# chzchzchz/raftsql

Measured on AMD Instinct MI355X. Metric: quorum decisions/sec (commit+vote) across G groups, higher is better.
Workload: dtype u64

## Files before the change

go/raftq/engine_more.go:

```go
package raftq

import "C"

import "unsafe"

func ABIVersion() int { return int(C.raftq_abi_version()) }

func Quorum(peers uint32) uint32 { return uint32(C.raftq_quorum(C.uint32_t(peers))) }

func (e *Engine) NGroups() uint64 { return uint64(C.raftq_groups(e.h)) }
func (e *Engine) NPeers() uint32  { return uint32(C.raftq_peers(e.h)) }

func (e *Engine) SelfMax() (int, error) {
	var slot C.int32_t
	if err := e.err(C.raftq_self_max(e.h, &slot)); err != nil {
		return -1, err
	}
	return int(slot), nil
}

func (e *Engine) Narrow() (bool, error) {
	var valid C.int32_t
	if err := e.err(C.raftq_narrow(e.h, &valid)); err != nil {
		return false, err
	}
	return valid != 0, nil
}

func (e *Engine) NarrowRebuild() error { return e.err(C.raftq_narrow_rebuild(e.h)) }

func (e *Engine) SetStream(stream unsafe.Pointer) error { return e.err(C.raftq_set_stream(e.h, stream)) }
func (e *Engine) Stream() unsafe.Pointer                { return C.raftq_get_stream(e.h) }

type TermDelta struct{ Group, CurTerm, FirstIdxCurTerm uint64 }

func (e *Engine) ApplyTermDeltas(d []TermDelta) error {
	if len(d) == 0 {
		return nil
	}
	return e.err(C.raftq_apply_term_deltas(e.h, (*C.raftq_term_delta_t)(unsafe.Pointer(&d[0])), C.uint64_t(len(d))))
}

func (e *Engine) CommitAdvance(gated bool, committedOut []uint64) (changed uint64, err error) {
	var p *C.uint64_t
	if committedOut != nil {
		p = (*C.uint64_t)(unsafe.Pointer(&committedOut[0]))
	}
	g := C.int(0)
	if gated {
		g = 1
	}
	var n C.uint64_t
	err = e.err(C.raftq_commit_advance(e.h, g, p, &n))
	return uint64(n), err
}

func (e *Engine) VoteTally(outcomeOut []uint8) (Counts, error) {
	var p *C.uint8_t
	if outcomeOut != nil {
		p = (*C.uint8_t)(unsafe.Pointer(&outcomeOut[0]))
	}
	var c C.raftq_counts_t
	if err := e.err(C.raftq_vote_tally(e.h, p, &c)); err != nil {
		return Counts{}, err
	}
	return Counts{uint64(c.n_changed), uint64(c.n_won), uint64(c.n_lost)}, nil
}

func (e *Engine) ReadVotes(out []uint8) error {
	return e.err(C.raftq_read_votes(e.h, (*C.uint8_t)(unsafe.Pointer(&out[0]))))
}

func (e *Engine) SetTimers(electionTick, heartbeatTick uint32, seed uint64) error {
	return e.err(C.raftq_set_timers(e.h, C.uint32_t(electionTick), C.uint32_t(heartbeatTick), C.uint64_t(seed)))
}

type TickCounts struct{ Hup, Beat uint64 }

func (e *Engine) Tick(wantCounts bool) (TickCounts, error) {
	var c C.raftq_tick_counts_t
	if !wantCounts {
		return TickCounts{}, e.err(C.raftq_tick(e.h, nil))
	}
	err := e.err(C.raftq_tick(e.h, &c))
	return TickCounts{uint64(c.n_hup), uint64(c.n_beat)}, err
}

func (e *Engine) CollectHups(out []uint64) (uint64, error) {
	var n C.uint64_t
	var p *C.uint64_t
	if len(out) > 0 {
		p = (*C.uint64_t)(unsafe.Pointer(&out[0]))
	}
	rc := C.raftq_collect_hups(e.h, p, C.uint64_t(len(out)), &n)
	return uint64(n), e.err(rc)
}

func (e *Engine) TickCollect(hups, beats []uint64) (nHup, nBeat uint64, err error) {
	var hp, bp *C.uint64_t
	if len(hups) > 0 {
		hp = (*C.uint64_t)(unsafe.Pointer(&hups[0]))
	}
	if len(beats) > 0 {
		bp = (*C.uint64_t)(unsafe.Pointer(&beats[0]))
	}
	var nh, nb C.uint64_t
	err = e.err(C.raftq_tick_collect(e.h, hp, C.uint64_t(len(hups)), &nh, bp, C.uint64_t(len(beats)), &nb))
	return uint64(nh), uint64(nb), err
}

const TickBeatBitmap = uint(C.RAFTQ_TICK_BEAT_BITMAP)

// ... 202 lines not shown
```

include/raftq.h:

```cpp
#ifndef RAFTQ_H
#define RAFTQ_H

#include <stddef.h>
#include <stdint.h>

#ifdef __cplusplus
extern "C" {
#endif

#define RAFTQ_ABI_VERSION 1
#define RAFTQ_MAX_PEERS 9

#define RAFTQ_OK 0
#define RAFTQ_EINVAL (-1)
#define RAFTQ_ENOMEM (-2)
#define RAFTQ_EHIP (-3)
#define RAFTQ_ESTATE (-4)
#define RAFTQ_ENODEV (-5)

#define RAFTQ_SWEEP_COMMIT 0x01u
#define RAFTQ_SWEEP_GATED 0x02u
#define RAFTQ_SWEEP_VOTES 0x04u
#define RAFTQ_SWEEP_NO_ADOPT 0x08u
#define RAFTQ_SWEEP_LDS 0x10u
// ... 16 lines not shown
  uint64_t match;
  uint32_t peer;
  uint32_t _pad;
} raftq_delta_t;

typedef struct raftq_vote_delta {
  uint64_t group;
  uint32_t peer;
  uint8_t vote;
  uint8_t _pad[3];
} raftq_vote_delta_t;

typedef struct raftq_term_delta {
  uint64_t group;
  uint64_t cur_term;
  uint64_t first_idx_cur_term;
} raftq_term_delta_t;

typedef struct raftq_advance {
  uint64_t group;
  uint64_t old_commit;
  uint64_t new_commit;
} raftq_advance_t;

typedef struct raftq_delta16 {
  uint64_t match;
  uint32_t group;
  uint32_t peer;
} raftq_delta16_t;
typedef struct raftq_advance16 {
  uint64_t new_commit;
  uint32_t group;
  uint32_t advanced_by;
} raftq_advance16_t;

int raftq_abi_version(void);
int raftq_device_count(int* n);
uint32_t raftq_quorum(uint32_t n_peers);

#define RAFTQ_MAX_GROUPS (1ull << 30)
int raftq_create(int device, uint64_t n_groups, uint32_t n_peers, raftq_t** out);
void raftq_destroy(raftq_t* h);
uint64_t raftq_groups(const raftq_t* h);
uint32_t raftq_peers(const raftq_t* h);
const char* raftq_last_error(const raftq_t* h);

int raftq_set_stream(raftq_t* h, void* stream);
void* raftq_get_stream(const raftq_t* h);

int raftq_load_match(raftq_t* h, const uint64_t* match ,
                     const uint64_t* committed );
int raftq_load_terms(raftq_t* h, const uint64_t* cur_term ,
                     const uint64_t* first_idx_cur_term );
int raftq_load_votes(raftq_t* h, const uint8_t* votes );

int raftq_apply_deltas(raftq_t* h, const raftq_delta_t* d, uint64_t n);
int raftq_apply_vote_deltas(raftq_t* h, const raftq_vote_delta_t* d, uint64_t n);
int raftq_apply_term_deltas(raftq_t* h, const raftq_term_delta_t* d, uint64_t n);

typedef struct raftq_voter_delta {
  uint64_t group;
  uint16_t voters;
  uint16_t reset;
  uint32_t _pad;
} raftq_voter_delta_t;
int raftq_load_voters(raftq_t* h, const uint16_t* voters);
int raftq_apply_voter_deltas(raftq_t* h, const raftq_voter_delta_t* d, uint64_t n);
int raftq_read_voters(raftq_t* h, uint16_t* voters_out);

int raftq_step_async(raftq_t* h, unsigned flags);
int raftq_wait(raftq_t* h, raftq_counts_t* counts);

int raftq_commit_advance(raftq_t* h, int gated, uint64_t* committed_out ,
                         uint64_t* n_changed );
int raftq_vote_tally(raftq_t* h, uint8_t* outcome_out ,
                     raftq_counts_t* counts );

int raftq_read_committed(raftq_t* h, uint64_t* committed_out );
int raftq_read_outcome(raftq_t* h, uint8_t* outcome_out );
int raftq_read_match(raftq_t* h, uint64_t* match_out );
int raftq_self_max(raftq_t* h, int32_t* slot_out);
int raftq_narrow(raftq_t* h, int32_t* valid_out);
int raftq_narrow_rebuild(raftq_t* h);
int raftq_read_votes(raftq_t* h, uint8_t* votes_out );
int raftq_collect_changed(raftq_t* h, raftq_advance_t* out, uint64_t cap, uint64_t* n);

#define RAFTQ_ROLE_FOLLOWER 0
#define RAFTQ_ROLE_CANDIDATE 1
#define RAFTQ_ROLE_LEADER 2
typedef struct raftq_tick_counts {
  uint64_t n_hup;
  uint64_t n_beat;
} raftq_tick_counts_t;
int raftq_set_timers(raftq_t* h, uint32_t election_tick, uint32_t heartbeat_tick, uint64_t seed);
int raftq_load_roles(raftq_t* h, const uint8_t* role , const uint32_t* elapsed );
int raftq_tick_set_voters(raftq_t* h, int on);
int raftq_tick(raftq_t* h, raftq_tick_counts_t* counts);
int raftq_read_tick(raftq_t* h, uint8_t* action , uint32_t* elapsed , uint8_t* role );
int raftq_collect_hups(raftq_t* h, uint64_t* groups, uint64_t cap, uint64_t* n);
int raftq_collect_beats(raftq_t* h, uint64_t* groups, uint64_t cap, uint64_t* n);
int raftq_tick_collect(raftq_t* h, uint64_t* hups, uint64_t hup_cap, uint64_t* n_hup, uint64_t* beats, uint64_t beat_cap,
                       uint64_t* n_beat);

#define RAFTQ_TICK_BEAT_BITMAP 1u
int raftq_tick_collect_lists(raftq_t* h, unsigned flags, uint64_t hup_cap, uint64_t beat_cap, uint64_t* n_hup, uint64_t* n_beat);
int raftq_last_tick_lists(raftq_t* h, const uint32_t** hups, uint64_t* n_hups, const uint32_t** beats, uint64_t* n_beats,
                          const uint64_t** beat_bitmap, uint64_t* bitmap_words);
int raftq_campaign(raftq_t* h, const uint64_t* groups, uint64_t n, uint32_t self_peer);

int raftq_cycle(raftq_t* h, const raftq_delta_t* deltas, uint64_t n_deltas,
                const raftq_vote_delta_t* vote_deltas, uint64_t n_vote_deltas, unsigned flags,
                raftq_advance_t* advances_out, uint64_t cap, uint64_t* n_advanced,
                raftq_counts_t* counts);

int raftq_stage(raftq_t* h, uint64_t n_deltas, uint64_t n_vote_deltas, raftq_delta_t** deltas,
                raftq_vote_delta_t** vote_deltas);
int raftq_last_advances(raftq_t* h, const raftq_advance_t** list, uint64_t* n_listed);

int raftq_cycle_packed(raftq_t* h, const raftq_delta16_t* deltas, uint64_t n_deltas,
                       const raftq_vote_delta_t* vote_deltas, uint64_t n_vote_deltas, unsigned flags,
                       raftq_advance16_t* advances_out, uint64_t cap, uint64_t* n_advanced,
                       raftq_counts_t* counts);
int raftq_stage_packed(raftq_t* h, uint64_t n_deltas, uint64_t n_vote_deltas, raftq_delta16_t** deltas,
                       raftq_vote_delta_t** vote_deltas);
int raftq_last_advances_packed(raftq_t* h, const raftq_advance16_t** list, uint64_t* n_listed);

#define RAFTQ_CYCLE_SEGMENTED 0x200u
int raftq_last_advance_segments(raftq_t* h, const raftq_advance16_t** recs, const uint32_t** counts, uint32_t* n_segments,
                                uint64_t* stride);

typedef struct raftq_set raftq_set_t;
#define RAFTQ_SET_GRID 0
#define RAFTQ_SET_PERSISTENT 1
int raftq_set_create(raftq_t* const* handles, uint32_t n, raftq_set_t** out);
void raftq_set_destroy(raftq_set_t* s);
uint32_t raftq_set_size(const raftq_set_t* s);
const char* raftq_set_last_error(const raftq_set_t* s);
void* raftq_set_get_stream(const raftq_set_t* s);
int raftq_set_mode(raftq_set_t* s, int mode, uint32_t persist_workgroups);
int raftq_set_sweep_async(raftq_set_t* s, unsigned flags);
int raftq_set_tick(raftq_set_t* s);
int raftq_set_wait(raftq_set_t* s, raftq_counts_t* per_member, raftq_counts_t* total);
int raftq_set_timer_begin(raftq_set_t* s);
int raftq_set_timer_end(raftq_set_t* s, float* elapsed_ms);
int raftq_sweep_many_async(raftq_t* const* handles, uint32_t n, unsigned flags);
int raftq_clone_state(raftq_t* dst, raftq_t* src);

int raftq_timer_begin(raftq_t* h);
int raftq_timer_end(raftq_t* h, float* elapsed_ms);

int raftq_host_alloc(void** p, uint64_t bytes);
void raftq_host_free(void* p);

#ifdef __cplusplus
}
#endif
#endif
```

raftsql_amd/_lib.py:

```python
from __future__ import annotations

import ctypes as C
import os

_HERE = os.path.dirname(os.path.abspath(__file__))
LIB_PATH = os.environ.get("RAFTQ_LIB") or os.path.join(_HERE, "libraftq.so")

RAFTQ_OK = 0
RAFTQ_EINVAL, RAFTQ_ENOMEM, RAFTQ_EHIP, RAFTQ_ESTATE, RAFTQ_ENODEV = -1, -2, -3, -4, -5

SWEEP_COMMIT = 0x01
SWEEP_GATED = 0x02
SWEEP_VOTES = 0x04
SWEEP_NO_ADOPT = 0x08
SWEEP_LDS = 0x10
SWEEP_CHANGED = 0x20
SWEEP_STREAM = 0x40
SWEEP_CACHED = 0x80
CYCLE_TRUSTED = 0x100
TICK_BEAT_BITMAP = 1
CYCLE_SEGMENTED = 0x200
SET_GRID, SET_PERSISTENT = 0, 1

MAX_PEERS = 9


class Counts(C.Structure):
    _fields_ = [("n_changed", C.c_uint64), ("n_won", C.c_uint64), ("n_lost", C.c_uint64)]


class TickCounts(C.Structure):
    _fields_ = [("n_hup", C.c_uint64), ("n_beat", C.c_uint64)]


class Delta(C.Structure):
    _fields_ = [("group", C.c_uint64), ("match", C.c_uint64), ("peer", C.c_uint32), ("_pad", C.c_uint32)]


class VoteDelta(C.Structure):
    _fields_ = [("group", C.c_uint64), ("peer", C.c_uint32), ("vote", C.c_uint8), ("_pad", C.c_uint8 * 3)]


class VoterDelta(C.Structure):
    _fields_ = [("group", C.c_uint64), ("voters", C.c_uint16), ("reset", C.c_uint16), ("_pad", C.c_uint32)]


class Advance(C.Structure):
    _fields_ = [("group", C.c_uint64), ("old_commit", C.c_uint64), ("new_commit", C.c_uint64)]


_H = C.c_void_p
_SIGS = [
    ("raftq_abi_version", C.c_int, []),
    ("raftq_device_count", C.c_int, [C.POINTER(C.c_int)]),
    ("raftq_quorum", C.c_uint32, [C.c_uint32]),
    ("raftq_create", C.c_int, [C.c_int, C.c_uint64, C.c_uint32, C.POINTER(_H)]),
    ("raftq_destroy", None, [_H]),
    ("raftq_groups", C.c_uint64, [_H]),
    ("raftq_peers", C.c_uint32, [_H]),
    ("raftq_last_error", C.c_char_p, [_H]),
    ("raftq_set_stream", C.c_int, [_H, C.c_void_p]),
    ("raftq_get_stream", C.c_void_p, [_H]),
    ("raftq_load_match", C.c_int, [_H, C.c_void_p, C.c_void_p]),
    ("raftq_load_terms", C.c_int, [_H, C.c_void_p, C.c_void_p]),
    ("raftq_load_votes", C.c_int, [_H, C.c_void_p]),
    ("raftq_apply_deltas", C.c_int, [_H, C.c_void_p, C.c_uint64]),
    ("raftq_apply_vote_deltas", C.c_int, [_H, C.c_void_p, C.c_uint64]),
    ("raftq_apply_term_deltas", C.c_int, [_H, C.c_void_p, C.c_uint64]),
    ("raftq_load_voters", C.c_int, [_H, C.c_void_p]),
    ("raftq_apply_voter_deltas", C.c_int, [_H, C.c_void_p, C.c_uint64]),
    ("raftq_read_voters", C.c_int, [_H, C.c_void_p]),
    ("raftq_step_async", C.c_int, [_H, C.c_uint]),
    ("raftq_wait", C.c_int, [_H, C.POINTER(Counts)]),
    ("raftq_commit_advance", C.c_int, [_H, C.c_int, C.c_void_p, C.POINTER(C.c_uint64)]),
    ("raftq_vote_tally", C.c_int, [_H, C.c_void_p, C.POINTER(Counts)]),
    ("raftq_read_committed", C.c_int, [_H, C.c_void_p]),
    ("raftq_read_outcome", C.c_int, [_H, C.c_void_p]),
    ("raftq_read_match", C.c_int, [_H, C.c_void_p]),
    ("raftq_self_max", C.c_int, [_H, C.POINTER(C.c_int32)]),
    ("raftq_narrow", C.c_int, [_H, C.POINTER(C.c_int32)]),
    ("raftq_narrow_rebuild", C.c_int, [_H]),
    ("raftq_read_votes", C.c_int, [_H, C.c_void_p]),
    ("raftq_collect_changed", C.c_int, [_H, C.c_void_p, C.c_uint64, C.POINTER(C.c_uint64)]),
    ("raftq_set_timers", C.c_int, [_H, C.c_uint32, C.c_uint32, C.c_uint64]),
    ("raftq_load_roles", C.c_int, [_H, C.c_void_p, C.c_void_p]),
    ("raftq_tick_set_voters", C.c_int, [_H, C.c_int]),
    ("raftq_tick", C.c_int, [_H, C.POINTER(TickCounts)]),
    ("raftq_read_tick", C.c_int, [_H, C.c_void_p, C.c_void_p, C.c_void_p]),
    ("raftq_collect_hups", C.c_int, [_H, C.c_void_p, C.c_uint64, C.POINTER(C.c_uint64)]),
    ("raftq_collect_beats", C.c_int, [_H, C.c_void_p, C.c_uint64, C.POINTER(C.c_uint64)]),
    ("raftq_tick_collect", C.c_int, [_H, C.c_void_p, C.c_uint64, C.POINTER(C.c_uint64), C.c_void_p, C.c_uint64, C.POINTER(C.c_uint64)]),
    ("raftq_tick_collect_lists", C.c_int, [_H, C.c_uint, C.c_uint64, C.c_uint64, C.POINTER(C.c_uint64), C.POINTER(C.c_uint64)]),
    ("raftq_last_tick_lists", C.c_int, [_H, C.POINTER(C.c_void_p), C.POINTER(C.c_uint64), C.POINTER(C.c_void_p), C.POINTER(C.c_uint64),
                                        C.POINTER(C.c_void_p), C.POINTER(C.c_uint64)]),
    ("raftq_campaign", C.c_int, [_H, C.c_void_p, C.c_uint64, C.c_uint32]),
    ("raftq_cycle", C.c_int, [_H, C.c_void_p, C.c_uint64, C.c_void_p, C.c_uint64, C.c_uint, C.c_void_p, C.c_uint64,
                              C.POINTER(C.c_uint64), C.POINTER(Counts)]),
    ("raftq_stage", C.c_int, [_H, C.c_uint64, C.c_uint64, C.POINTER(C.c_void_p), C.POINTER(C.c_void_p)]),
    ("raftq_last_advances", C.c_int, [_H, C.POINTER(C.c_void_p), C.POINTER(C.c_uint64)]),
    ("raftq_cycle_packed", C.c_int, [_H, C.c_void_p, C.c_uint64, C.c_void_p, C.c_uint64, C.c_uint, C.c_void_p, C.c_uint64,
                                     C.POINTER(C.c_uint64), C.POINTER(Counts)]),
    ("raftq_stage_packed", C.c_int, [_H, C.c_uint64, C.c_uint64, C.POINTER(C.c_void_p), C.POINTER(C.c_void_p)]),
    ("raftq_last_advances_packed", C.c_int, [_H, C.POINTER(C.c_void_p), C.POINTER(C.c_uint64)]),
    ("raftq_last_advance_segments", C.c_int, [_H, C.POINTER(C.c_void_p), C.POINTER(C.c_void_p), C.POINTER(C.c_uint32), C.POINTER(C.c_uint64)]),
    ("raftq_set_create", C.c_int, [C.POINTER(_H), C.c_uint32, C.POINTER(_H)]),
    ("raftq_set_destroy", None, [_H]),
    ("raftq_set_size", C.c_uint32, [_H]),
    ("raftq_set_last_error", C.c_char_p, [_H]),
    ("raftq_set_get_stream", C.c_void_p, [_H]),
    ("raftq_set_mode", C.c_int, [_H, C.c_int, C.c_uint32]),
    ("raftq_set_sweep_async", C.c_int, [_H, C.c_uint]),
    ("raftq_set_wait", C.c_int, [_H, C.c_void_p, C.POINTER(Counts)]),
    ("raftq_set_tick", C.c_int, [_H]),
    ("raftq_set_timer_begin", C.c_int, [_H]),
    ("raftq_set_timer_end", C.c_int, [_H, C.POINTER(C.c_float)]),
    ("raftq_sweep_many_async", C.c_int, [C.POINTER(_H), C.c_uint32, C.c_uint]),
    ("raftq_clone_state", C.c_int, [_H, _H]),
    ("raftq_timer_begin", C.c_int, [_H]),
    ("raftq_timer_end", C.c_int, [_H, C.POINTER(C.c_float)]),
    ("raftq_host_alloc", C.c_int, [C.POINTER(C.c_void_p), C.c_uint64]),
    ("raftq_host_free", None, [C.c_void_p]),
]
EXPORTS = [s[0] for s in _SIGS]


class StepCounts(C.Structure):
    _fields_ = [("n_msgs", C.c_uint64), ("n_groups_touched", C.c_uint64)]


_STEP_SIGS = [
    ("raftq_set_self", C.c_int, [_H, C.c_uint32]),
    ("raftq_load_node", C.c_int, [_H, C.c_void_p, C.c_void_p, C.c_void_p, C.c_void_p, C.c_void_p]),
    ("raftq_read_node", C.c_int, [_H, C.c_void_p, C.c_void_p, C.c_void_p, C.c_void_p, C.c_void_p, C.c_void_p]),
    ("raftq_step_batch", C.c_int, [_H, C.c_void_p, C.c_uint64, C.c_void_p, C.POINTER(StepCounts)]),
    ("raftq_apply_log_deltas", C.c_int, [_H, C.c_void_p, C.c_uint64, C.c_void_p]),
    ("raftq_apply_log_deltas_nowait", C.c_int, [_H, C.c_void_p, C.c_uint64]),
    ("raftq_step_submit", C.c_int, [_H, C.c_void_p, C.c_uint64]),
    ("raftq_step_collect", C.c_int, [_H, C.c_void_p, C.POINTER(StepCounts)]),
    ("raftq_step_stage", C.c_int, [_H, C.c_uint64, C.POINTER(C.c_void_p)]),
    ("raftq_step_stage_packed", C.c_int, [_H, C.c_uint64, C.POINTER(C.c_void_p)]),
    ("raftq_step_submit_packed", C.c_int, [_H, C.c_void_p, C.c_uint64]),
    ("raftq_step_results", C.c_int, [_H, C.POINTER(C.c_void_p), C.POINTER(C.c_uint64)]),
    ("raftq_step_set_compact", C.c_int, [_H, C.c_int]),
    ("raftq_step_set_msg_flags", C.c_int, [_H, C.c_int]),
    ("raftq_step_set_voters", C.c_int, [_H, C.c_int]),
    ("raftq_step_results_c", C.c_int, [_H, C.POINTER(C.c_void_p), C.POINTER(C.c_uint64)]),
    ("raftq_step_results_s", C.c_int, [_H, C.POINTER(C.c_void_p), C.POINTER(C.c_uint64)]),
]
STEP_EXPORTS = [s[0] for s in _STEP_SIGS]



class WireCounts(C.Structure):
    _fields_ = [("n_msgs", C.c_uint64), ("n_ents", C.c_uint64), ("n_malformed", C.c_uint64), ("bytes", C.c_uint64)]


class WalCounts(C.Structure):
    _fields_ = [("n_recs", C.c_uint64), ("n_valid", C.c_uint64), ("bytes", C.c_uint64), ("last_crc", C.c_uint32),
                ("_pad", C.c_uint32)]


_WIRE_SIGS = [
    ("raftq_wire_encode", C.c_int, [_H, C.c_void_p, C.c_uint64, C.c_void_p, C.c_uint64, C.c_void_p, C.c_uint64, C.c_void_p,
                                    C.c_uint64, C.c_void_p, C.POINTER(WireCounts)]),
# ... 67 lines not shown
```

raftsql_amd/csrc/raftq_capi.hip:

```cpp
#include "raftq.h"

#include <hip/hip_runtime.h>

#include <algorithm>
#include <atomic>
#include <mutex>
#include <chrono>
#include <cstdlib>
#include <cstdio>
#include <cstring>
#include <new>
#include <string>
#include <unordered_set>
#include <vector>

#include "raftq_internal.hpp"

#ifndef RAFTQ_GPL
#define RAFTQ_GPL 4
#endif
#ifndef RAFTQ_AUTO_STREAM_BYTES
#define RAFTQ_AUTO_STREAM_BYTES (128ull << 20)
#endif
#ifndef RAFTQ_LDS_GPL
// ... 134 lines not shown
template <int N>
hipError_t launch_voters_n(const VoterSweepArgs& a, uint64_t gpad, unsigned flags, int nt, hipStream_t s) {
  const bool commit = flags & (RAFTQ_SWEEP_COMMIT | RAFTQ_SWEEP_GATED);
  const bool gated = flags & RAFTQ_SWEEP_GATED;
  const bool votes = flags & RAFTQ_SWEEP_VOTES;
  if (commit && gated) return votes ? launch_voters_reg<N, true, true, true>(a, gpad, nt, s) : launch_voters_reg<N, true, true, false>(a, gpad, nt, s);
  if (commit) return votes ? launch_voters_reg<N, true, false, true>(a, gpad, nt, s) : launch_voters_reg<N, true, false, false>(a, gpad, nt, s);
  return launch_voters_reg<N, false, false, true>(a, gpad, nt, s);
}

hipError_t launch_voters(uint32_t N, const VoterSweepArgs& a, uint64_t gpad, unsigned flags, int nt, hipStream_t s) {
  switch (N) {
    case 1: return launch_voters_n<1>(a, gpad, flags, nt, s);
    case 2: return launch_voters_n<2>(a, gpad, flags, nt, s);
    case 3: return launch_voters_n<3>(a, gpad, flags, nt, s);
    case 4: return launch_voters_n<4>(a, gpad, flags, nt, s);
    case 5: return launch_voters_n<5>(a, gpad, flags, nt, s);
    case 6: return launch_voters_n<6>(a, gpad, flags, nt, s);
    case 7: return launch_voters_n<7>(a, gpad, flags, nt, s);
    case 8: return launch_voters_n<8>(a, gpad, flags, nt, s);
    case 9: return launch_voters_n<9>(a, gpad, flags, nt, s);
    default: return hipErrorInvalidValue;
  }
}

hipError_t launch_sweep(uint32_t N, const SweepLaunch& L, unsigned flags, int nt, hipStream_t s) {
  switch (N) {
    case 1: return launch_n<1>(L, flags, nt, s);
    case 2: return launch_n<2>(L, flags, nt, s);
    case 3: return launch_n<3>(L, flags, nt, s);
    case 4: return launch_n<4>(L, flags, nt, s);
    case 5: return launch_n<5>(L, flags, nt, s);
    case 6: return launch_n<6>(L, flags, nt, s);
    case 7: return launch_n<7>(L, flags, nt, s);
    case 8: return launch_n<8>(L, flags, nt, s);
    case 9: return launch_n<9>(L, flags, nt, s);
    default: return hipErrorInvalidValue;
  }
}

}
static inline void dense_changed(raftq_t* h) { h->node_mirror_fresh = false; }

int raftq_detail::ensure_staging(raftq_t* h, size_t bytes) {
  HIPCHK(h, h->stage.grow(bytes, std::max({bytes, h->stage.cap * 2, (size_t)1 << 20}), &h->stream));
  return RAFTQ_OK;
}

int raftq_detail::ensure_ingest(raftq_t* h, size_t bytes) {
  HIPCHK(h, h->ingest.grow(bytes, std::max({bytes, h->ingest.cap * 2, (size_t)1 << 20}), &h->stream, h->bar));
  return RAFTQ_OK;
}

namespace {
int ensure_adv(raftq_t* h, uint64_t entries) {
  const uint64_t have = h->adv.cap / sizeof(Advance);
  const uint64_t want = std::min<uint64_t>(std::max<uint64_t>({entries, have * 2, 4096}), h->gpad);
  HIPCHK(h, h->adv.grow(entries * sizeof(Advance), want * sizeof(Advance), &h->stream));
  return RAFTQ_OK;
}

}
int raftq_detail::self_max_check(raftq_t* h) {
  if (int rc = use_device(h)) return rc;
  if (h->step_collected != h->step_submitted) {
    HIPCHK(h, hipMemsetAsync(h->self_max, 0, sizeof(uint32_t), h->stream));
    return RAFTQ_OK;
  }
  HIPCHK(h, hipMemsetD32Async((hipDeviceptr_t)h->self_max, (int)(kSelfMaxValid | h->self_peer), 1, h->stream));
  const uint64_t blocks = std::min<uint64_t>((h->G + kBlock - 1) / kBlock, 4096);
  hipLaunchKernelGGL(self_max_check_kernel, dim3((unsigned)std::max<uint64_t>(blocks, 1)), dim3(kBlock), 0, h->stream,
                     (const uint64_t*)h->match, h->ld, h->G, h->N, h->self_peer, h->self_max);
  HIPCHK(h, hipGetLastError());
  return RAFTQ_OK;
}
int raftq_detail::narrow_build(raftq_t* h) {
  if (int rc = use_device(h)) return rc;
  if (h->narrow_off) return RAFTQ_OK;
  if (h->step_collected != h->step_submitted) {
    HIPCHK(h, hipMemsetAsync(h->narrow_word(), 0, sizeof(uint32_t), h->stream));
    return RAFTQ_OK;
  }
  if (!h->anchor) {
    const hipError_t e = raftq_buf::alloc_group({{(void**)&h->anchor, h->ld * sizeof(uint64_t)},
                                                 {(void**)&h->moff, (size_t)h->N * h->ld * sizeof(uint32_t)}},
                                                h->stream);
    if (e != hipSuccess) {
      (void)hipGetLastError();
      return RAFTQ_OK;
    }
    if (h->in_set) h->in_set->tab_stale = true;
  }
  HIPCHK(h, hipMemsetD32Async((hipDeviceptr_t)h->narrow_word(), (int)kNarrowValid, 1, h->stream));
  const uint64_t blocks = std::min<uint64_t>((h->G + kBlock - 1) / kBlock, 4096);
  hipLaunchKernelGGL(narrow_build_kernel, dim3((unsigned)std::max<uint64_t>(blocks, 1)), dim3(kBlock), 0, h->stream,
                     (const uint64_t*)h->match, h->ld, h->G, h->N, h->anchor, h->moff, h->narrow_word());
  HIPCHK(h, hipGetLastError());
  return RAFTQ_OK;
}
int raftq_detail::use_device(raftq_t* h) {
  if (!h) return fail(nullptr, RAFTQ_EINVAL, "null handle");
  HIPCHK(h, hipSetDevice(h->device));
  return RAFTQ_OK;
}
int raftq_detail::use_device_idle(raftq_t* h, const char* who) {
  if (int rc = use_device(h)) return rc;
  if (h->step_collected != h->step_submitted)
    return fail(h, RAFTQ_ESTATE, std::string(who) + ": Step batches are in flight; collect them first");
  return RAFTQ_OK;
}
using raftq_detail::ensure_staging;
using raftq_detail::ensure_ingest;
using raftq_detail::use_device;
using raftq_detail::use_device_idle;
using raftq_detail::ensure_tick_state;

template <typename W>
static void pack_votes(const uint8_t* votes, uint64_t G, uint32_t N, W* out) {
  for (uint64_t g = 0; g < G; ++g) out[g] = 0;
  for (uint32_t p = 0; p < N; ++p) {
    const uint8_t* row = votes + (size_t)p * G;
    for (uint64_t g = 0; g < G; ++g) {
      const uint8_t v = row[g];
      out[g] = (W)(out[g] | (W)((v == 1 ? 1u : v == 2 ? 2u : 0u) << (2 * p)));
    }
  }
}
template <typename W>
static void unpack_votes(const W* in, uint64_t G, uint32_t N, uint8_t* votes) {
  for (uint32_t p = 0; p < N; ++p) {
    uint8_t* row = votes + (size_t)p * G;
    for (uint64_t g = 0; g < G; ++g) {
      const uint32_t f = ((uint32_t)in[g] >> (2 * p)) & 3u;
      row[g] = f == 3u ? 0 : (uint8_t)f;
    }
  }
}

extern "C" {

int raftq_abi_version(void) { return RAFTQ_ABI_VERSION; }

uint32_t raftq_quorum(uint32_t n_peers) { return n_peers / 2 + 1; }

int raftq_device_count(int* n) {
  if (!n) return fail(nullptr, RAFTQ_EINVAL, "raftq_device_count: null out");
  int c = 0;
  hipError_t e = hipGetDeviceCount(&c);
  if (e != hipSuccess) {
    *n = 0;
    return fail(nullptr, RAFTQ_ENODEV, std::string("hipGetDeviceCount: ") + hipGetErrorString(e));
  }
  *n = c;
  return RAFTQ_OK;
}

const char* raftq_last_error(const raftq_t* h) { return h ? h->err.c_str() : g_err.c_str(); }

uint64_t raftq_groups(const raftq_t* h) { return h ? h->G : 0; }
uint32_t raftq_peers(const raftq_t* h) { return h ? h->N : 0; }

int raftq_create(int device, uint64_t n_groups, uint32_t n_peers, raftq_t** out) {
  if (!out) return fail(nullptr, RAFTQ_EINVAL, "raftq_create: null out");
  *out = nullptr;
  if (n_groups == 0 || n_groups > RAFTQ_MAX_GROUPS)
    return fail(nullptr, RAFTQ_EINVAL, "raftq_create: n_groups out of range (1 .. RAFTQ_MAX_GROUPS = 2^30 per handle)");
  if (n_peers < 1 || n_peers > RAFTQ_MAX_PEERS) return fail(nullptr, RAFTQ_EINVAL, "raftq_create: n_peers must be 1..9");
  int ndev = 0;
  if (hipGetDeviceCount(&ndev) != hipSuccess || ndev <= 0)
    return fail(nullptr, RAFTQ_ENODEV, "raftq_create: no HIP device (this library has no CPU path)");
  if (device < 0 || device >= ndev) return fail(nullptr, RAFTQ_ENODEV, "raftq_create: device index out of range");
  raftq_t* h = new (std::nothrow) raftq();
  if (!h) return fail(nullptr, RAFTQ_ENOMEM, "raftq_create: host allocation failed");
  h->device = device;
  h->G = n_groups;
  h->N = n_peers;
  h->last_gpl = kGPL;
  h->gpad = (n_groups + kTileMax - 1) / kTileMax * kTileMax;
  h->ld = h->gpad + kRowStagger;
  const uint64_t ld = h->ld;
  h->max_partials = h->gpad / (kBlock * 2) * kWaves;
  int rc = RAFTQ_OK;
  do {
    if ((rc = use_device(h))) break;
    hipError_t e = hipStreamCreateWithFlags(&h->stream, hipStreamNonBlocking);
    if (e != hipSuccess) { rc = fail(h, RAFTQ_EHIP, std::string("hipStreamCreate: ") + hipGetErrorString(e)); break; }
    h->own_stream = true;
    {
      int large_bar = 0;
      (void)hipDeviceGetAttribute(&large_bar, hipDeviceAttributeIsLargeBar, device);
      const char* st = std::getenv("RAFTQ_STAGE");
      h->bar.staging = large_bar == 1 && !(st && std::strcmp(st, "host") == 0);
    }
    e = raftq_buf::alloc_group({{(void**)&h->match, (size_t)n_peers * ld * 8},
                                {(void**)&h->committed[0], ld * 8},
                                {(void**)&h->committed[1], ld * 8},
                                {(void**)&h->first_idx, ld * 8},
                                {(void**)&h->votes, (size_t)vote_word_bytes((int)n_peers) * ld},
                                {(void**)&h->outcome, ld / 4 + 64},
                                {(void**)&h->changed_bits, h->gpad / 8},
                                {(void**)&h->partials, h->max_partials * sizeof(uint4)},
                                {(void**)&h->offsets, (h->max_partials + 1) * 8},
                                {(void**)&h->self_max, 64}},
                               h->stream);
    if (e != hipSuccess) {
      rc = fail(h, e == hipErrorOutOfMemory ? RAFTQ_ENOMEM : RAFTQ_EHIP, std::string("device arrays: ") + hipGetErrorString(e));
      break;
    }
    {
      const char* nr = std::getenv("RAFTQ_NARROW");
      h->narrow_off = nr && std::strcmp(nr, "0") == 0;
    }
    e = hipMemsetD32Async((hipDeviceptr_t)h->self_max, (int)(kSelfMaxValid | 0u), 1, h->stream);
    if (e != hipSuccess) { rc = fail(h, RAFTQ_EHIP, std::string("hipMemsetD32Async: ") + hipGetErrorString(e)); break; }
    e = raftq_buf::alloc_group({{(void**)&h->h_partials, h->max_partials * sizeof(uint4), raftq_buf::Kind::pinned},
                                {(void**)&h->h_total, 64, raftq_buf::Kind::mapped_coherent, (void**)&h->d_total}},
                               h->stream);
    if (e != hipSuccess) { rc = fail(h, RAFTQ_ENOMEM, std::string("page-locked memory: ") + hipGetErrorString(e)); break; }
    e = hipEventCreate(&h->ev0);
    if (e == hipSuccess) e = hipEventCreate(&h->ev1);
    if (e != hipSuccess) { rc = fail(h, RAFTQ_EHIP, std::string("hipEventCreate: ") + hipGetErrorString(e)); break; }
    e = hipStreamSynchronize(h->stream);
    if (e != hipSuccess) { rc = fail(h, RAFTQ_EHIP, std::string("hipStreamSynchronize: ") + hipGetErrorString(e)); break; }
  } while (0);
  if (rc != RAFTQ_OK) {
    std::string keep = h->err;
    raftq_destroy(h);
    g_err = keep;
    return rc;
  }
  *out = h;
  return RAFTQ_OK;
}

void raftq_destroy(raftq_t* h) {
  if (!h) return;
  if (h->in_set) {
    raftq_set_t* s = h->in_set;
    s->broken = true;
    s->members.erase(std::remove(s->members.begin(), s->members.end(), h), s->members.end());
    (void)hipSetDevice(h->device);
    (void)hipStreamSynchronize(s->stream);
    h->stream = nullptr;
    h->own_stream = false;
  }
  if (h->prof_n && std::getenv("RAFTQ_PROFILE"))
    std::fprintf(stderr,
                 "[raftq] cycle phases, avg us over %llu calls: stage/validate %.1f | enqueue scatter %.1f | enqueue sweep "
                 "%.1f | enqueue collect %.1f | sync %.1f | copy-out %.1f | turns that ended in the blocking wait instead of the "
                 "polled flag: %llu\n",
                 (unsigned long long)h->prof_n, h->prof[0] / h->prof_n, h->prof[1] / h->prof_n, h->prof[2] / h->prof_n,
                 h->prof[3] / h->prof_n, h->prof[4] / h->prof_n, h->prof[5] / h->prof_n, (unsigned long long)h->flag_fallbacks);
  (void)hipSetDevice(h->device);
  if (h->stream) (void)hipStreamSynchronize(h->stream);
  if (h->many_aux) (void)hipStreamSynchronize(h->many_aux);
  raftq_detail::free_node_state(h);
  raftq_detail::free_wire_state(h);
  raftq_buf::free_device(h->match, h->committed[0], h->committed[1], h->first_idx, h->votes, h->voters, h->outcome, h->changed_bits,
                         h->partials, h->offsets, h->self_max, h->anchor, h->moff, h->claim, h->delta_bad, h->role, h->elapsed, h->action, h->hup_bits,
                         h->beat_bits, h->tick_partials, h->tick_offsets2);
  raftq_buf::free_host(h->h_partials, h->h_total);
  if (h->ev0) (void)hipEventDestroy(h->ev0);
  if (h->ev1) (void)hipEventDestroy(h->ev1);
  if (h->many_aux) {
    (void)hipEventDestroy(h->many_fork);
    (void)hipEventDestroy(h->many_join);
  }
  const hipStream_t streams[4] = {h->many_aux, h->step_s_in, h->step_s_out, h->own_stream ? h->stream : nullptr};
  delete h;
  for (hipStream_t st : streams)
    if (st) (void)hipStreamDestroy(st);
}

int raftq_set_stream(raftq_t* h, void* stream) {
  if (int rc = use_device_idle(h, "raftq_set_stream")) return rc;
  if (h->in_set) return fail(h, RAFTQ_ESTATE, "raftq_set_stream: the handle is a member of a sweep set, which owns its stream");
  HIPCHK(h, hipStreamSynchronize(h->stream));
  if (h->own_stream) HIPCHK(h, hipStreamDestroy(h->stream));
  h->stream = (hipStream_t)stream;
  h->own_stream = false;
  return RAFTQ_OK;
}

void* raftq_get_stream(const raftq_t* h) { return h ? (void*)h->stream : nullptr; }

int raftq_load_match(raftq_t* h, const uint64_t* match, const uint64_t* committed) {
  if (int rc = use_device_idle(h, "raftq_load_match")) return rc;
  if (!match && !committed) return fail(h, RAFTQ_EINVAL, "raftq_load_match: nothing to load");
  if (match) {
    for (uint32_t p = 0; p < h->N; ++p)
      HIPCHK(h, hipMemcpyAsync(h->match + (size_t)p * h->ld, match + (size_t)p * h->G, h->G * 8, hipMemcpyHostToDevice, h->stream));
    if (int rc = raftq_detail::self_max_check(h)) return rc;
    if (int rc = raftq_detail::narrow_build(h)) return rc;
  }
  dense_changed(h);
  if (committed)
    HIPCHK(h, hipMemcpyAsync(h->committed[h->cur], committed, h->G * 8, hipMemcpyHostToDevice, h->stream));
  HIPCHK(h, hipStreamSynchronize(h->stream));
  return RAFTQ_OK;
}

int raftq_load_terms(raftq_t* h, const uint64_t* cur_term, const uint64_t* first_idx_cur_term) {
  if (int rc = use_device_idle(h, "raftq_load_terms")) return rc;
  if (!cur_term || !first_idx_cur_term) return fail(h, RAFTQ_EINVAL, "raftq_load_terms: null argument");
  std::vector<uint64_t> f;
  try {
    f.assign(first_idx_cur_term, first_idx_cur_term + h->G);
  } catch (...) {
    return fail(h, RAFTQ_ENOMEM, "raftq_load_terms: host allocation failed");
  }
  for (uint64_t g = 0; g < h->G; ++g)
    if (cur_term[g] == 0) f[g] = 0;
  HIPCHK(h, hipMemcpyAsync(h->first_idx, f.data(), h->G * 8, hipMemcpyHostToDevice, h->stream));
  dense_changed(h);
  HIPCHK(h, hipStreamSynchronize(h->stream));
  h->have_terms = true;
  return RAFTQ_OK;
}

int raftq_load_votes(raftq_t* h, const uint8_t* votes) {
  if (int rc = use_device_idle(h, "raftq_load_votes")) return rc;
  if (!votes) return fail(h, RAFTQ_EINVAL, "raftq_load_votes: null argument");
  const size_t wb = (size_t)vote_word_bytes((int)h->N);
  std::vector<uint8_t> packed;
  try {
    packed.resize(h->G * wb);
  } catch (...) {
    return fail(h, RAFTQ_ENOMEM, "raftq_load_votes: host allocation failed");
  }
  if (wb == 2) pack_votes(votes, h->G, h->N, reinterpret_cast<uint16_t*>(packed.data()));
  else pack_votes(votes, h->G, h->N, reinterpret_cast<uint32_t*>(packed.data()));
  HIPCHK(h, hipMemcpyAsync(h->votes, packed.data(), packed.size(), hipMemcpyHostToDevice, h->stream));
  HIPCHK(h, hipStreamSynchronize(h->stream));
  return RAFTQ_OK;
}

static int ensure_delta_dev(raftq_t* h, size_t bytes) {
  if (!h->delta_bad) HIPCHK(h, raftq_buf::alloc_zeroed((void**)&h->delta_bad, 64, h->stream));
  HIPCHK(h, h->delta_dev.grow(bytes, std::max(bytes * 2, (size_t)1 << 20), &h->stream));
  return RAFTQ_OK;
}

static int check_deltas(raftq_t* h, bool trusted = false) {
  int rc = RAFTQ_OK;
  const char* what = trusted ? "; that record was dropped, every other record of the turn was applied (RAFTQ_CYCLE_TRUSTED)"
                             : "; nothing applied";
  if (h->delta_check[0] && h->h_total[1] == h->delta_check[0])
    rc = fail(h, RAFTQ_EINVAL, std::string("a match delta is out of range (group >= G or peer >= N)") + what);
  if (h->delta_check[1] && h->h_total[2] == h->delta_check[1])
    rc = fail(h, RAFTQ_EINVAL, std::string("a vote delta is invalid (group/peer out of range or vote not 1/2)") + what);
  h->delta_check[0] = h->delta_check[1] = 0;
  return rc;
}

}

template <typename Rec, typename AbiRec>
static int enqueue_ingest(raftq_t* h, const AbiRec* d, uint64_t n, const raftq_vote_delta_t* vd, uint64_t nv, size_t off_votes,
                          bool trusted = false) {
  static_assert(sizeof(Rec) == sizeof(AbiRec), "ABI struct mismatch");
  static_assert(sizeof(VoteDeltaRec) == sizeof(raftq_vote_delta_t), "ABI struct mismatch");
  if (nv > 0xfffffffeull) return fail(h, RAFTQ_EINVAL, "vote delta batch too large");
  auto inside = [&](const void* q) {
    return (const uint8_t*)q >= (const uint8_t*)h->ingest.h && (const uint8_t*)q < (const uint8_t*)h->ingest.h + h->ingest.cap;
  };
  if (n) {
    AbiRec* dst = (AbiRec*)h->ingest.h;
    if ((const void*)d != (const void*)dst) {
      if (inside(d)) return fail(h, RAFTQ_EINVAL, "match deltas staged with other counts / another record layout than this call's");
      std::memcpy(dst, d, (size_t)n * sizeof(AbiRec));
    }
  }
  if (nv) {
    raftq_vote_delta_t* dst = (raftq_vote_delta_t*)((uint8_t*)h->ingest.h + off_votes);
    if ((const void*)vd != (const void*)dst) {
      if (inside(vd)) return fail(h, RAFTQ_EINVAL, "vote deltas staged with other counts / another record layout than this call's");
      std::memcpy(dst, vd, (size_t)nv * sizeof(raftq_vote_delta_t));
    }
    if (!h->claim) {
      HIPCHK(h, raftq_buf::alloc_filled((void**)&h->claim, (size_t)h->N * h->ld * sizeof(uint32_t), 0xff, h->stream));
    }
  }
  h->ingest.publish();
  if (int rc = ensure_delta_dev(h, h->ingest.cap)) return rc;
  const unsigned long long em = n ? ++h->delta_epoch : kNoEpoch, ev = nv ? ++h->delta_epoch : kNoEpoch;
  h->delta_check[0] = n ? em : 0;
  h->delta_check[1] = nv ? ev : 0;
  Rec* dev_m = (Rec*)h->delta_dev.d;
  VoteDeltaRec* dev_v = (VoteDeltaRec*)((uint8_t*)h->delta_dev.d + off_votes);
  const unsigned long long* bad = h->delta_bad;
  const dim3 gm((unsigned)((n + kBlock - 1) / kBlock)), gv((unsigned)((nv + kBlock - 1) / kBlock));
  if (n) dense_changed(h);
  if (n && trusted)
    hipLaunchKernelGGL((deltas_in_apply_kernel<Rec>), gm, dim3(kBlock), 0, h->stream, (const Rec*)h->ingest.d, n, h->match, h->ld,
                       h->G, h->N, h->delta_bad, h->d_total + 1, em, h->self_max, h->narrow_mirror());
  else if (n)
    hipLaunchKernelGGL((deltas_in_kernel<Rec>), gm, dim3(kBlock), 0, h->stream, (const Rec*)h->ingest.d, dev_m, n, h->G, h->N,
                       h->delta_bad, h->d_total + 1, em);
  if (nv)
    hipLaunchKernelGGL(vote_deltas_in_kernel, gv, dim3(kBlock), 0, h->stream,
                       (const VoteDeltaRec*)((uint8_t*)h->ingest.d + off_votes), dev_v, nv, h->G, h->N, h->delta_bad + 1,
                       h->d_total + 2, ev);
  if (n && !trusted)
    hipLaunchKernelGGL((apply_deltas_kernel<Rec>), gm, dim3(kBlock), 0, h->stream, h->match, h->ld, (const Rec*)dev_m, n, bad, em,
                       ev, h->self_max, h->narrow_mirror());
  if (nv) {
    const unsigned long long em_gate = trusted ? kNoEpoch : em;
    hipLaunchKernelGGL(vote_claim_kernel, gv, dim3(kBlock), 0, h->stream, h->claim, h->ld, (const VoteDeltaRec*)dev_v, nv, bad,
                       em_gate, ev, h->G, h->N, trusted ? 1 : 0);
    hipLaunchKernelGGL(vote_apply_kernel, gv, dim3(kBlock), 0, h->stream, h->votes, h->N > 8 ? 1 : 0, h->claim, h->ld,
                       (const VoteDeltaRec*)dev_v, nv, bad, em_gate, ev, h->G, h->N, trusted ? 1 : 0);
  }
  HIPCHK(h, hipGetLastError());
  return RAFTQ_OK;
}

extern "C" {

int raftq_apply_deltas(raftq_t* h, const raftq_delta_t* d, uint64_t n) {
  if (int rc = use_device_idle(h, "raftq_apply_deltas")) return rc;
  if (n == 0) return RAFTQ_OK;
  if (!d) return fail(h, RAFTQ_EINVAL, "raftq_apply_deltas: null argument");
  if (int rc = ensure_ingest(h, (size_t)n * sizeof(raftq_delta_t))) return rc;
  if (int rc = enqueue_ingest<DeltaRec>(h, d, n, nullptr, 0, 0)) return rc;
  HIPCHK(h, hipStreamSynchronize(h->stream));
  return check_deltas(h);
}

int raftq_apply_term_deltas(raftq_t* h, const raftq_term_delta_t* d, uint64_t n) {
  static_assert(sizeof(TermDeltaRec) == sizeof(raftq_term_delta_t), "ABI struct mismatch");
  if (int rc = use_device_idle(h, "raftq_apply_term_deltas")) return rc;
  if (n == 0) return RAFTQ_OK;
  if (!d) return fail(h, RAFTQ_EINVAL, "raftq_apply_term_deltas: null argument");
  for (uint64_t i = 0; i < n; ++i)
    if (d[i].group >= h->G) return fail(h, RAFTQ_EINVAL, "a term delta is out of range; nothing applied");
  if (int rc = ensure_staging(h, (size_t)n * sizeof(raftq_term_delta_t))) return rc;
  raftq_term_delta_t* dst = (raftq_term_delta_t*)h->stage.h;
  uint64_t m = 0;
  {
    std::unordered_set<uint64_t> seen;
    seen.reserve((size_t)n * 2);
    std::vector<uint64_t> keep;
    keep.reserve(n);
    for (uint64_t i = n; i-- > 0;)
      if (seen.insert(d[i].group).second) keep.push_back(i);
    for (auto it = keep.rbegin(); it != keep.rend(); ++it) dst[m++] = d[*it];
  }
  const dim3 grid((unsigned)((m + kBlock - 1) / kBlock));
  dense_changed(h);
  hipLaunchKernelGGL(apply_term_deltas_kernel, grid, dim3(kBlock), 0, h->stream, h->first_idx,
                     (const TermDeltaRec*)h->stage.d, m);
  HIPCHK(h, hipGetLastError());
  HIPCHK(h, hipStreamSynchronize(h->stream));
  h->have_terms = true;
  return RAFTQ_OK;
}

int raftq_apply_vote_deltas(raftq_t* h, const raftq_vote_delta_t* d, uint64_t n) {
  if (int rc = use_device_idle(h, "raftq_apply_vote_deltas")) return rc;
  if (n == 0) return RAFTQ_OK;
  if (!d) return fail(h, RAFTQ_EINVAL, "raftq_apply_vote_deltas: null argument");
  if (int rc = ensure_ingest(h, (size_t)n * sizeof(raftq_vote_delta_t))) return rc;
  if (int rc = enqueue_ingest<DeltaRec>(h, (const raftq_delta_t*)nullptr, 0, d, n, 0)) return rc;
  HIPCHK(h, hipStreamSynchronize(h->stream));
  return check_deltas(h);
}

}

static int ensure_voters(raftq_t* h) {
  if (h->voters) return RAFTQ_OK;
  HIPCHK(h, raftq_buf::alloc_zeroed((void**)&h->voters, h->ld * sizeof(uint16_t), h->stream));
  return RAFTQ_OK;
}
static int drop_voters(raftq_t* h) {
  if (!h->voters) return RAFTQ_OK;
  HIPCHK(h, hipStreamSynchronize(h->stream));
  raftq_buf::free_device(h->voters);
  return RAFTQ_OK;
}
static int voters_not_in_set(raftq_t* h, const char* who) {
  if (!h->in_set) return RAFTQ_OK;
  return fail(h, RAFTQ_ESTATE, std::string(who) + ": the handle is a member of a sweep set, whose dispatches count every slot "
                                                  "(voter masks on set members are out of scope)");
}
int raftq_detail::refuse_voters(raftq_t* h, const char* who, bool step_family, bool tick_rounds, bool bcast) {
  if (!h || !h->voters) return RAFTQ_OK;
  if (tick_rounds && h->tick_voters) return RAFTQ_OK;
  if (bcast) {
    if (h->bcast_voters) return RAFTQ_OK;
    return fail(h, RAFTQ_ESTATE, std::string(who) + ": the handle has voter masks loaded and did not opt in with raftq_bcast_set_voters; its broadcast "
                                                    "would go to N - 1 slots, not to a group's membership (whatever raftq_step_set_voters and "
                                                    "raftq_tick_set_voters say)");
  }
  if (h->step_voters) {
    if (step_family) return RAFTQ_OK;
    return fail(h, RAFTQ_ESTATE, std::string(who) + ": the handle has voter masks loaded; the broadcasts built on the device go to N - 1 slots, "
                                                    "not to a group's membership (out of scope, whatever raftq_step_set_voters says)");
  }
  return fail(h, RAFTQ_ESTATE, std::string(who) + ": the handle has voter masks loaded; Step's maybeCommit / poll on the device "
                                                  "count every slot (out of scope: raftq_load_voters(h, NULL) first)");
}

extern "C" {

int raftq_load_voters(raftq_t* h, const uint16_t* voters) {
  if (int rc = use_device_idle(h, "raftq_load_voters")) return rc;
  if (int rc = voters_not_in_set(h, "raftq_load_voters")) return rc;
  if (!voters) return drop_voters(h);
  const uint32_t beyond = 0xffffu & ~((1u << h->N) - 1u);
  for (uint64_t g = 0; g < h->G; ++g)
    if (voters[g] & beyond) return fail(h, RAFTQ_EINVAL, "raftq_load_voters: a mask names a peer slot >= N; nothing loaded");
  if (int rc = ensure_voters(h)) return rc;
  HIPCHK(h, hipMemcpyAsync(h->voters, voters, h->G * sizeof(uint16_t), hipMemcpyHostToDevice, h->stream));
  HIPCHK(h, hipStreamSynchronize(h->stream));
  return RAFTQ_OK;
}

int raftq_read_voters(raftq_t* h, uint16_t* voters_out) {
  if (int rc = use_device_idle(h, "raftq_read_voters")) return rc;
  if (!voters_out) return fail(h, RAFTQ_EINVAL, "raftq_read_voters: null argument");
  if (!h->voters) {
    std::fill(voters_out, voters_out + h->G, (uint16_t)((1u << h->N) - 1u));
    return RAFTQ_OK;
  }
  HIPCHK(h, hipMemcpyAsync(voters_out, h->voters, h->G * sizeof(uint16_t), hipMemcpyDeviceToHost, h->stream));
  HIPCHK(h, hipStreamSynchronize(h->stream));
  return RAFTQ_OK;
}

int raftq_apply_voter_deltas(raftq_t* h, const raftq_voter_delta_t* d, uint64_t n) {
  static_assert(sizeof(VoterDeltaRec) == sizeof(raftq_voter_delta_t), "ABI struct mismatch");
  if (int rc = use_device_idle(h, "raftq_apply_voter_deltas")) return rc;
  if (int rc = voters_not_in_set(h, "raftq_apply_voter_deltas")) return rc;
// ... 134 lines not shown
    return RAFTQ_OK;
  }
  raftq_t* h0 = handles[0];
  if (int rc = use_device(h0)) return rc;
  if (!h0->many_aux) {
    HIPCHK(h0, hipStreamCreateWithFlags(&h0->many_aux, hipStreamNonBlocking));
    HIPCHK(h0, hipEventCreateWithFlags(&h0->many_fork, hipEventDisableTiming));
    HIPCHK(h0, hipEventCreateWithFlags(&h0->many_join, hipEventDisableTiming));
  }
  HIPCHK(h0, hipEventRecord(h0->many_fork, h0->stream));
  HIPCHK(h0, hipStreamWaitEvent(h0->many_aux, h0->many_fork, 0));
  int rc = RAFTQ_OK;
  for (uint32_t i = 0; i < n && rc == RAFTQ_OK; ++i)
    rc = sweep_on(handles[i], flags, (i & 1) ? h0->many_aux : h0->stream, "raftq_sweep_many_async");
  HIPCHK(h0, hipEventRecord(h0->many_join, h0->many_aux));
  HIPCHK(h0, hipStreamWaitEvent(h0->stream, h0->many_join, 0));
  return rc;
}

int raftq_wait(raftq_t* h, raftq_counts_t* counts) {
  if (int rc = use_device_idle(h, "raftq_wait")) return rc;
  if (counts) {
    if (h->n_partials == 0) return fail(h, RAFTQ_ESTATE, "raftq_wait: no sweep to report on");
    HIPCHK(h, hipMemcpyAsync(h->h_partials, h->partials, h->n_partials * sizeof(uint4), hipMemcpyDeviceToHost, h->stream));
  }
  HIPCHK(h, hipStreamSynchronize(h->stream));
  if (counts) {
    uint64_t c = 0, w = 0, l = 0;
    for (uint64_t i = 0; i < h->n_partials; ++i) {
      c += h->h_partials[i].x;
      w += h->h_partials[i].y;
      l += h->h_partials[i].z;
    }
    const bool commit = h->last_flags & (RAFTQ_SWEEP_COMMIT | RAFTQ_SWEEP_GATED);
    const bool votes = h->last_flags & RAFTQ_SWEEP_VOTES;
    counts->n_changed = commit ? c : 0;
    counts->n_won = votes ? w : 0;
    counts->n_lost = votes ? l : 0;
  }
  return RAFTQ_OK;
}

int raftq_read_committed(raftq_t* h, uint64_t* out) {
  if (int rc = use_device_idle(h, "raftq_read_committed")) return rc;
  if (!out) return fail(h, RAFTQ_EINVAL, "raftq_read_committed: null argument");
  const uint64_t* src = (h->last_flags & RAFTQ_SWEEP_NO_ADOPT) && h->last_new ? h->last_new : h->committed[h->cur];
  HIPCHK(h, hipMemcpyAsync(out, src, h->G * 8, hipMemcpyDeviceToHost, h->stream));
  HIPCHK(h, hipStreamSynchronize(h->stream));
  return RAFTQ_OK;
}

int raftq_read_outcome(raftq_t* h, uint8_t* out) {
  if (int rc = use_device_idle(h, "raftq_read_outcome")) return rc;
  if (!out) return fail(h, RAFTQ_EINVAL, "raftq_read_outcome: null argument");
  std::vector<uint8_t> packed;
  try {
    packed.resize((h->G + 3) / 4);
  } catch (...) {
    return fail(h, RAFTQ_ENOMEM, "raftq_read_outcome: host allocation failed");
  }
  HIPCHK(h, hipMemcpyAsync(packed.data(), h->outcome, packed.size(), hipMemcpyDeviceToHost, h->stream));
  HIPCHK(h, hipStreamSynchronize(h->stream));
  for (uint64_t g = 0; g < h->G; ++g) out[g] = (uint8_t)((packed[g >> 2] >> (2 * (g & 3))) & 3u);
  return RAFTQ_OK;
}

int raftq_self_max(raftq_t* h, int32_t* slot) {
  if (int rc = use_device_idle(h, "raftq_self_max")) return rc;
  if (!slot) return fail(h, RAFTQ_EINVAL, "raftq_self_max: null argument");
  uint32_t w = 0;
  HIPCHK(h, hipMemcpyAsync(&w, h->self_max, sizeof w, hipMemcpyDeviceToHost, h->stream));
  HIPCHK(h, hipStreamSynchronize(h->stream));
  *slot = (w & kSelfMaxValid) ? (int32_t)(w & 0xffu) : -1;
  return RAFTQ_OK;
}

int raftq_narrow(raftq_t* h, int32_t* valid) {
  if (int rc = use_device_idle(h, "raftq_narrow")) return rc;
  if (!valid) return fail(h, RAFTQ_EINVAL, "raftq_narrow: null argument");
  uint32_t w = 0;
  HIPCHK(h, hipMemcpyAsync(&w, h->narrow_word(), sizeof w, hipMemcpyDeviceToHost, h->stream));
  HIPCHK(h, hipStreamSynchronize(h->stream));
  *valid = w == kNarrowValid ? 1 : 0;
  return RAFTQ_OK;
}

int raftq_narrow_rebuild(raftq_t* h) {
  if (int rc = use_device_idle(h, "raftq_narrow_rebuild")) return rc;
  if (int rc = raftq_detail::narrow_build(h)) return rc;
  HIPCHK(h, hipStreamSynchronize(h->stream));
  return RAFTQ_OK;
}

int raftq_read_match(raftq_t* h, uint64_t* out) {
  if (int rc = use_device_idle(h, "raftq_read_match")) return rc;
  if (!out) return fail(h, RAFTQ_EINVAL, "raftq_read_match: null argument");
  for (uint32_t p = 0; p < h->N; ++p)
    HIPCHK(h, hipMemcpyAsync(out + (size_t)p * h->G, h->match + (size_t)p * h->ld, h->G * 8, hipMemcpyDeviceToHost, h->stream));
  HIPCHK(h, hipStreamSynchronize(h->stream));
  return RAFTQ_OK;
}

int raftq_read_votes(raftq_t* h, uint8_t* out) {
  if (int rc = use_device_idle(h, "raftq_read_votes")) return rc;
  if (!out) return fail(h, RAFTQ_EINVAL, "raftq_read_votes: null argument");
  const size_t wb = (size_t)vote_word_bytes((int)h->N);
  std::vector<uint8_t> packed;
  try {
    packed.resize(h->G * wb);
  } catch (...) {
    return fail(h, RAFTQ_ENOMEM, "raftq_read_votes: host allocation failed");
  }
  HIPCHK(h, hipMemcpyAsync(packed.data(), h->votes, packed.size(), hipMemcpyDeviceToHost, h->stream));
  HIPCHK(h, hipStreamSynchronize(h->stream));
  if (wb == 2) unpack_votes(reinterpret_cast<const uint16_t*>(packed.data()), h->G, h->N, out);
  else unpack_votes(reinterpret_cast<const uint32_t*>(packed.data()), h->G, h->N, out);
  return RAFTQ_OK;
}

int raftq_commit_advance(raftq_t* h, int gated, uint64_t* committed_out, uint64_t* n_changed) {
  if (int rc = raftq_step_async(h, gated ? (RAFTQ_SWEEP_COMMIT | RAFTQ_SWEEP_GATED) : RAFTQ_SWEEP_COMMIT)) return rc;
  raftq_counts_t c;
  if (int rc = raftq_wait(h, &c)) return rc;
  if (n_changed) *n_changed = c.n_changed;
  if (committed_out) return raftq_read_committed(h, committed_out);
  return RAFTQ_OK;
}

int raftq_vote_tally(raftq_t* h, uint8_t* outcome_out, raftq_counts_t* counts) {
  if (int rc = raftq_step_async(h, RAFTQ_SWEEP_VOTES)) return rc;
  raftq_counts_t c;
  if (int rc = raftq_wait(h, &c)) return rc;
  if (counts) *counts = c;
  if (outcome_out) return raftq_read_outcome(h, outcome_out);
  return RAFTQ_OK;
}

}

int raftq_detail::ensure_tick_state(raftq_t* h) {
  if (h->role) return RAFTQ_OK;
  HIPCHK(h, raftq_buf::alloc_group({{(void**)&h->role, h->ld},
                                    {(void**)&h->elapsed, h->ld * 4},
                                    {(void**)&h->action, h->ld},
                                    {(void**)&h->hup_bits, h->gpad / 8},
                                    {(void**)&h->beat_bits, h->gpad / 8},
                                    {(void**)&h->tick_partials, h->gpad / 256 * sizeof(uint4)}},
                                   h->stream));
  return RAFTQ_OK;
}

static int ensure_tick_offsets2(raftq_t* h, uint64_t nw);
static hipError_t wait_turn(raftq_t* h, uint64_t flag_epoch, int kind = 0);

extern "C" {

int raftq_set_timers(raftq_t* h, uint32_t election_tick, uint32_t heartbeat_tick, uint64_t seed) {
  if (!h) return fail(nullptr, RAFTQ_EINVAL, "null handle");
  if (election_tick == 0 || heartbeat_tick == 0)
    return fail(h, RAFTQ_EINVAL, "raftq_set_timers: ticks must be >= 1");
  h->election_tick = election_tick;
  h->heartbeat_tick = heartbeat_tick;
  h->tick_seed = seed;
  return RAFTQ_OK;
}

// ... 899 lines not shown
  for (raftq_t* h : s->members) {
    h->tl_valid = false;
    ++h->tick_no;
    h->ticked = true;
  }
  return RAFTQ_OK;
}

int raftq_set_wait(raftq_set_t* s, raftq_counts_t* per_member, raftq_counts_t* total) {
  if (int rc = set_ready(s, "raftq_set_wait")) return rc;
  const bool want = per_member || total;
  const size_t n = s->members.size();
  if (want) {
    if (!s->swept) return sfail(s, RAFTQ_ESTATE, "raftq_set_wait: no set sweep to report on");
    set_fill_table(s, -1, s->tab_host);
    SETCHK(s, hipMemcpyAsync(s->tab[2], s->tab_host.data(), n * sizeof(SweepArgs), hipMemcpyHostToDevice, s->stream));
    s->np_host.resize(n);
    for (size_t i = 0; i < n; ++i) s->np_host[i] = s->members[i]->n_partials;
    SETCHK(s, hipMemcpyAsync(s->np_d, s->np_host.data(), n * 8, hipMemcpyHostToDevice, s->stream));
    hipLaunchKernelGGL(set_counts_kernel, dim3((unsigned)n), dim3(kBlock), 0, s->stream, (const SweepArgs*)s->tab[2],
                       (const uint64_t*)s->np_d, s->counts_d);
    SETCHK(s, hipGetLastError());
    SETCHK(s, hipMemcpyAsync(s->counts_h, s->counts_d, n * 32, hipMemcpyDeviceToHost, s->stream));
  }
  SETCHK(s, hipStreamSynchronize(s->stream));
  if (want) {
    raftq_counts_t t{0, 0, 0};
    for (size_t i = 0; i < n; ++i) {
      const unsigned f = s->members[i]->last_flags;
      const bool commit = f & (RAFTQ_SWEEP_COMMIT | RAFTQ_SWEEP_GATED);
      const bool votes = f & RAFTQ_SWEEP_VOTES;
      raftq_counts_t c{commit ? s->counts_h[4 * i] : 0, votes ? s->counts_h[4 * i + 1] : 0, votes ? s->counts_h[4 * i + 2] : 0};
      if (per_member) per_member[i] = c;
      t.n_changed += c.n_changed;
      t.n_won += c.n_won;
      t.n_lost += c.n_lost;
    }
    if (total) *total = t;
  }
  return RAFTQ_OK;
}

int raftq_set_timer_begin(raftq_set_t* s) {
  if (int rc = set_ready(s, "raftq_set_timer_begin")) return rc;
  SETCHK(s, hipEventRecord(s->ev0, s->stream));
  return RAFTQ_OK;
}

int raftq_set_timer_end(raftq_set_t* s, float* elapsed_ms) {
  if (int rc = set_ready(s, "raftq_set_timer_end")) return rc;
  if (!elapsed_ms) return sfail(s, RAFTQ_EINVAL, "raftq_set_timer_end: null argument");
  SETCHK(s, hipEventRecord(s->ev1, s->stream));
  SETCHK(s, hipEventSynchronize(s->ev1));
  SETCHK(s, hipEventElapsedTime(elapsed_ms, s->ev0, s->ev1));
  return RAFTQ_OK;
}

int raftq_clone_state(raftq_t* dst, raftq_t* src) {
  if (int rc = use_device_idle(dst, "raftq_clone_state")) return rc;
  if (!src) return fail(dst, RAFTQ_EINVAL, "raftq_clone_state: null source");
  if (src == dst) return RAFTQ_OK;
  if (src->device != dst->device || src->N != dst->N || src->G != dst->G)
    return fail(dst, RAFTQ_EINVAL, "raftq_clone_state: source and destination must have the same device, groups and peers");
  if (src->step_collected != src->step_submitted)
    return fail(dst, RAFTQ_ESTATE, "raftq_clone_state: the source has Step batches in flight");
  if (src->voters && dst->in_set)
    return fail(dst, RAFTQ_ESTATE, "raftq_clone_state: the source has voter masks loaded and the destination is a member of a sweep "
                                   "set, whose dispatches count every slot (out of scope)");
  if (src->voters) {
    if (int rc = ensure_voters(dst)) return rc;
  } else if (int rc = drop_voters(dst)) {
    return rc;
  }
  HIPCHK(dst, hipStreamSynchronize(src->stream));
  const uint64_t ld = dst->ld;
  HIPCHK(dst, hipMemcpyAsync(dst->match, src->match, (size_t)dst->N * ld * 8, hipMemcpyDeviceToDevice, dst->stream));
  HIPCHK(dst, hipMemcpyAsync(dst->committed[dst->cur], src->committed[src->cur], ld * 8, hipMemcpyDeviceToDevice, dst->stream));
  HIPCHK(dst, hipMemcpyAsync(dst->first_idx, src->first_idx, ld * 8, hipMemcpyDeviceToDevice, dst->stream));
  HIPCHK(dst, hipMemcpyAsync(dst->votes, src->votes, (size_t)vote_word_bytes((int)dst->N) * ld, hipMemcpyDeviceToDevice,
                             dst->stream));
  HIPCHK(dst, hipMemcpyAsync(dst->self_max, src->self_max, sizeof(uint32_t), hipMemcpyDeviceToDevice, dst->stream));
  if (src->anchor && !dst->narrow_off && !dst->anchor) {
    if (raftq_buf::alloc_group({{(void**)&dst->anchor, ld * sizeof(uint64_t), raftq_buf::Kind::device, nullptr, false},
                                {(void**)&dst->moff, (size_t)dst->N * ld * sizeof(uint32_t), raftq_buf::Kind::device, nullptr, false}},
                               dst->stream) != hipSuccess)
      (void)hipGetLastError();
    else if (dst->in_set) dst->in_set->tab_stale = true;
  }
  if (src->anchor && dst->anchor && !dst->narrow_off) {
    HIPCHK(dst, hipMemcpyAsync(dst->anchor, src->anchor, ld * sizeof(uint64_t), hipMemcpyDeviceToDevice, dst->stream));
    HIPCHK(dst, hipMemcpyAsync(dst->moff, src->moff, (size_t)dst->N * ld * sizeof(uint32_t), hipMemcpyDeviceToDevice, dst->stream));
    HIPCHK(dst, hipMemcpyAsync(dst->narrow_word(), src->narrow_word(), sizeof(uint32_t), hipMemcpyDeviceToDevice, dst->stream));
  } else {
    HIPCHK(dst, hipMemsetAsync(dst->narrow_word(), 0, sizeof(uint32_t), dst->stream));
  }
  if (src->voters) HIPCHK(dst, hipMemcpyAsync(dst->voters, src->voters, ld * sizeof(uint16_t), hipMemcpyDeviceToDevice, dst->stream));
  HIPCHK(dst, hipStreamSynchronize(dst->stream));
  dst->have_terms = src->have_terms;
  dense_changed(dst);
  return RAFTQ_OK;
}

}
```

raftsql_amd/csrc/raftq_internal.hpp:

```cpp
#pragma once
#include <hip/hip_runtime.h>

#include <string>
#include <vector>

#include "raftq.h"
#include "raftq_wire.h"
#include "raftq_kernels.hpp"
#include "raftq_buffers.hpp"

struct raftq {
  int device = 0;
  uint64_t G = 0, gpad = 0, ld = 0;
  uint32_t N = 0;
  hipStream_t stream = nullptr;
  bool own_stream = false;
  struct raftq_set* in_set = nullptr;
  uint64_t* match = nullptr;
  uint64_t* committed[2] = {nullptr, nullptr};
  int cur = 0;
  uint64_t* first_idx = nullptr;
  uint8_t* votes = nullptr;
  uint16_t* voters = nullptr;
  uint8_t* outcome = nullptr;
  uint64_t* changed_bits = nullptr;
  uint4* partials = nullptr;
  uint4* h_partials = nullptr;
  uint64_t n_partials = 0;
  uint64_t max_partials = 0;
  uint64_t* offsets = nullptr;
  uint64_t* h_total = nullptr;
  raftq_buf::Buffer<> stage{raftq_buf::Kind::mapped};
  raftq_buf::HostWritable ingest;
  raftq_buf::BarRule bar;
  std::vector<uint64_t> ld_mark, ld_start;
  struct LdNowait {
    raftq_buf::Buffer<> buf{raftq_buf::Kind::mapped};
    hipEvent_t ev = nullptr;
  };
  LdNowait ld_nowait[2];
  uint32_t ld_nowait_next = 0;
  std::vector<uint32_t> ld_round, ld_pos;
  uint32_t ld_epoch = 0;
  raftq_buf::Buffer<raftqk::Advance> adv{raftq_buf::Kind::mapped_coherent};
  uint64_t adv_listed = 0;
  bool adv_packed = false;
  bool adv_segmented = false;
  raftq_buf::Buffer<uint32_t> seg_h{raftq_buf::Kind::mapped_coherent};
  raftq_buf::Buffer<unsigned int> seg_d{raftq_buf::Kind::device};
  uint32_t seg_tiles = 0, seg_stride = 0, seg_one = 0;
  uint64_t flag_mask = ~0ull;
  uint32_t* self_max = nullptr;
  uint64_t* anchor = nullptr;
  uint32_t* moff = nullptr;
  bool narrow_off = false;
  uint32_t* narrow_word() const { return self_max + 1; }
  raftqk::NarrowMirror narrow_mirror() const { return raftqk::NarrowMirror{self_max + 1, anchor, moff}; }
  uint64_t compact_epoch = 0;
  uint64_t compact_epoch_armed = 0;
  uint32_t flag_misses[2] = {0, 0}, flag_rested[2] = {0, 0};
  uint64_t flag_fallbacks = 0;
  uint32_t* claim = nullptr;
  raftq_buf::Buffer<> delta_dev{raftq_buf::Kind::device};
  unsigned long long* delta_bad = nullptr;
  unsigned long long delta_epoch = 0;
  unsigned long long delta_check[2] = {0, 0};
  uint8_t* role = nullptr;
  uint32_t* elapsed = nullptr;
  uint8_t* action = nullptr;
  uint64_t* hup_bits = nullptr;
  uint64_t* beat_bits = nullptr;
  uint4* tick_partials = nullptr;
  raftq_buf::Buffer<uint32_t> tl{raftq_buf::Kind::mapped_coherent};
  uint64_t tl_hup_cap = 0, tl_beat_cap = 0, tl_beat_at = 0, tl_map_off = 0;
  uint64_t tl_n_hup = 0, tl_n_beat = 0;
  unsigned tl_flags = 0;
  bool tl_valid = false;
  uint64_t* tick_offsets2 = nullptr;
  uint32_t election_tick = 10, heartbeat_tick = 1;
  uint64_t tick_seed = 0x1000, tick_no = 0;
  bool ticked = false;
  uint64_t* d_total = nullptr;
  bool have_terms = false;
  unsigned last_flags = 0;
  int last_gpl = 0;
  const uint64_t* last_old = nullptr;
  const uint64_t* last_new = nullptr;
  uint32_t self_peer = 0;
  bool self_set = false;
  bool node_mirror_fresh = false;
  uint64_t node_mirror_refreshes = 0;
  void* node_rec = nullptr;
  unsigned int* step_stall = nullptr;
  uint8_t step_compact = 0;
  bool step_msg_flags = false;
  bool step_voters = false;
  bool tick_voters = false;
  bool bcast_voters = false;
  int step_walk_mode = 1;
  uint32_t step_stalls_in_a_row = 0, step_sorted_left = 0;
  uint64_t step_replays = 0;
  static constexpr int kStepSlots = 3;
  struct StepSlot {
    raftq_buf::Buffer<> in_h{raftq_buf::Kind::pinned};
    raftq_buf::HostWritable in_bar;
    raftq_buf::Buffer<> dev{raftq_buf::Kind::device};
    raftq_buf::Buffer<> out{raftq_buf::Kind::mapped};
    uint64_t n = 0;
    hipEvent_t ev_in = nullptr, ev_out = nullptr;
    bool busy = false;
    bool lists = false;
    bool replayed = false;
    bool copy_pending = false;
    const void* w_off_in_place = nullptr;
    const void* w_stream_in_place = nullptr;
    size_t w_stage_stream_off = 0;
    const void* msgs_in_place = nullptr;
    const void* outs_d = nullptr;
    uint64_t out_quads = 0;
    int end_bit = 0;
    uint32_t rec = 64;
    bool tail_zeroed = false;
    uint64_t tail_n = 0;
    uint32_t tail_rec = 0;
    const void* tail_dev = nullptr;
    uint64_t w_nbytes = 0;
    bool wire = false;
    uint8_t recs = 0;
    void* w_msgs_d = nullptr;
    void* w_ents_d = nullptr;
    const uint64_t* w_ent_total_d = nullptr;
    uint64_t w_ents_cap = 0;
    raftq_buf::Buffer<> w_pin{raftq_buf::Kind::pinned};
    bool w_msgs_fetched = false, w_ents_fetched = false;
    uint64_t w_n_ents = 0;
  } step_slot[kStepSlots];
  int step_last_slot = -1;
  uint64_t step_submitted = 0, step_collected = 0;
  hipStream_t step_s_in = nullptr, step_s_out = nullptr;
  bool step_defer_copy = true;
  const void* step_last_out = nullptr;
  uint64_t step_last_n = 0;
  uint32_t step_last_rec = 64;
  hipEvent_t ev0 = nullptr, ev1 = nullptr;
  hipStream_t many_aux = nullptr;
  hipEvent_t many_fork = nullptr, many_join = nullptr;
  raftq_buf::Buffer<> wire_dev{raftq_buf::Kind::device};
  raftq_buf::Buffer<> wire_out{raftq_buf::Kind::device};
  uint64_t* wire_pin = nullptr;
  uint64_t* wire_pin_d = nullptr;
  unsigned long long* wire_flags = nullptr;
  raftq_buf::Buffer<unsigned long long> wire_lb{raftq_buf::Kind::device};
  uint64_t wire_lb_tiles = 0;
  uint32_t wire_ticket_base = 0, wire_epoch = 0;
  uint32_t wire_chunk_base = 0, wire_chunk_pending = 0;
  bool wire_chunk_unknown = false;
  unsigned int prop_stamp = 0;
  raftq_buf::Buffer<> resp_dev{raftq_buf::Kind::device};
  bool resp_on = false;
  uint32_t resp_stamp = 0;
  const uint64_t* resp_at_tail_d = nullptr;
  bool wal_pending = false, wal_pending_done = false;
  bool wal_pending_waited = false;
  uint64_t wal_pending_n = 0, wal_pending_cap = 0;
  uint32_t wal_pending_prev = 0;
  int wal_pending_rc = 0;
  raftq_wal_counts_t wal_pending_counts{};
  std::string wal_pending_err;
  std::string err;
  double prof[6] = {0, 0, 0, 0, 0, 0};
  uint64_t prof_n = 0;
};


struct raftq_set {
  int device = 0;
  uint32_t N = 0;
  uint64_t gpad = 0;
  std::vector<raftq_t*> members;
  hipStream_t stream = nullptr;
  raftqk::SweepArgs* tab[3] = {nullptr, nullptr, nullptr};
  std::vector<raftqk::SweepArgs> tab_host;
  uint64_t* counts_d = nullptr;
  uint64_t* np_d = nullptr;
  std::vector<uint64_t> np_host;
  uint64_t* counts_h = nullptr;
  bool swept = false;
  bool broken = false;
  bool tab_stale = false;
  unsigned last_flags = 0;
  int mode = 0;
  uint32_t persist_wgs = 0;
  hipEvent_t ev0 = nullptr, ev1 = nullptr;
  raftqk::TickArgs* tick_tab = nullptr;
  std::vector<raftqk::TickArgs> tick_host;
  uint64_t tick_since = 0;
  std::string err;
};


struct raftq_wire_counts;
namespace raftqk {
struct NodeArrays;
}
namespace raftq_detail {
int node_arrays_of(raftq_t* h, raftqk::NodeArrays* out);
int fail(raftq_t* h, int code, const std::string& msg);
int use_device(raftq_t* h);
int use_device_idle(raftq_t* h, const char* who);
int refuse_voters(raftq_t* h, const char* who, bool step_family = false, bool tick_rounds = false, bool bcast = false);
inline bool masked_tick(const raftq_t* h) { return h->voters != nullptr && h->tick_voters; }
inline bool masked_bcast(const raftq_t* h) { return h->voters != nullptr && h->bcast_voters; }
int self_max_check(raftq_t* h);
int narrow_build(raftq_t* h);
int ensure_staging(raftq_t* h, size_t bytes);
int ensure_ingest(raftq_t* h, size_t bytes);
int ensure_tick_state(raftq_t* h);
void free_node_state(raftq_t* h);
void free_wire_state(raftq_t* h);
struct PackedDst {
  int form;
  uint32_t head_types;
  void* wide;
  uint64_t wide_cap;
};
int wire_frames_enqueue(raftq_t* h, const void* stream, uint64_t nbytes, const uint64_t* frame_off, uint64_t n, void* msgs, void* ents,
                        uint64_t ents_cap, void* msgs_d, int tail_appends, void* zero2 ,
                        const PackedDst* packed = nullptr);
uint64_t wire_frames_n_wide(raftq_t* h);
int wire_frames_finish(raftq_t* h, const uint64_t* frame_off, uint64_t n, bool have_ents, uint64_t ents_cap, ::raftq_wire_counts* counts);
struct RespPlan {
  uint64_t n = 0, n_max = 0, cap = 0;
  void* v_out = nullptr;
  uint64_t* v_resp_off = nullptr;
  uint64_t* peer_off = nullptr;
};
int respond_prepare(raftq_t* h, const void* stream, uint64_t nbytes, const uint64_t* frame_off, const void* msgs, const void* ents,
                    const uint64_t* at_tail, void* out, uint64_t cap, uint64_t* resp_off, uint64_t* peer_off, uint64_t n, RespPlan* p);
int respond_enqueue(raftq_t* h, const RespPlan& p);
int respond_finish(raftq_t* h, const RespPlan& p, ::raftq_wire_counts* resp_counts);
struct TickLists {
  unsigned flags;
  uint64_t cap_h, cap_b, beat_at, map_off;
  const uint64_t* off_beat;
  const uint64_t* off_h = nullptr;
};
int tick_lists_prepare(raftq_t* h, const char* who, unsigned flags, uint64_t hup_cap, uint64_t beat_cap, TickLists* tl);
int tick_lists_enqueue(raftq_t* h, TickLists* tl);
int tick_lists_finish(raftq_t* h, const char* who, const TickLists& tl, uint64_t* n_hup, uint64_t* n_beat);
int node_records_of(raftq_t* h, const char* who, raftqk::NodeArrays* out, bool tick_rounds = false, bool bcast = false);
int respond_pass_ok(raftq_t* h);
hipError_t wait_call(raftq_t* h);
}

#define HIPCHK(h, expr)                                                                        \
  do {                                                                                         \
    hipError_t _e = (expr);                                                                    \
    if (_e != hipSuccess) {                                                                    \
      return raftq_detail::fail((h), _e == hipErrorOutOfMemory ? RAFTQ_ENOMEM : RAFTQ_EHIP,    \
                                std::string(#expr) + ": " + hipGetErrorString(_e));            \
    }                                                                                          \
  } while (0)
```

raftsql_amd/csrc/raftq_kernels.hpp:

```cpp
#pragma once
#include <hip/hip_runtime.h>
#include <stdint.h>

#include <utility>

namespace raftqk {

typedef unsigned long long u64x2 __attribute__((ext_vector_type(2)));

constexpr int kBlock = 256;
constexpr int kWaves = kBlock / 64;
constexpr int kMaxPeers = 9;
constexpr int kTileMax = 2048;

struct SweepArgs {
  const uint64_t* match;
  const uint64_t* committed;
  uint64_t* committed_out;
  const uint64_t* first_idx;
  const uint8_t* votes;
  uint8_t* outcome;
  uint64_t* changed_bits;
  uint4* partials;
  uint64_t ld;
  const uint32_t* self_max = nullptr;
  const uint32_t* narrow = nullptr;
  const uint64_t* anchor = nullptr;
  const uint32_t* moff = nullptr;
};

constexpr uint32_t kSelfMaxValid = 0x80000000u;

constexpr uint32_t kNarrowValid = 1u;

template <typename T>
__device__ __forceinline__ void ce_desc(T& a, T& b) {
  const bool gt = a > b;
  const T hi = gt ? a : b;
  const T lo = gt ? b : a;
  a = hi;
  b = lo;
}

template <int N, typename T = uint64_t>
__device__ __forceinline__ T select_quorum_network(T (&v)[N]) {
#define CE(i, j) ce_desc(v[i], v[j])
  if constexpr (N == 2) { CE(0, 1); }
  if constexpr (N == 3) { CE(0, 2); CE(0, 1); CE(1, 2); }
  if constexpr (N == 4) { CE(0, 2); CE(1, 3); CE(0, 1); CE(2, 3); CE(1, 2); }
  if constexpr (N == 5) {
    CE(0, 3); CE(1, 4); CE(0, 2); CE(1, 3); CE(0, 1); CE(2, 4); CE(1, 2); CE(3, 4); CE(2, 3);
  }
  if constexpr (N == 6) {
    CE(0, 5); CE(1, 3); CE(2, 4); CE(1, 2); CE(3, 4); CE(0, 3);
    CE(2, 5); CE(0, 1); CE(2, 3); CE(4, 5); CE(1, 2); CE(3, 4);
  }
  if constexpr (N == 7) {
    CE(0, 6); CE(2, 3); CE(4, 5); CE(0, 2); CE(1, 4); CE(3, 6); CE(0, 1); CE(2, 5);
    CE(3, 4); CE(1, 2); CE(4, 6); CE(2, 3); CE(4, 5); CE(1, 2); CE(3, 4); CE(5, 6);
  }
  if constexpr (N == 8) {
    CE(0, 2); CE(1, 3); CE(4, 6); CE(5, 7); CE(0, 4); CE(1, 5); CE(2, 6); CE(3, 7); CE(0, 1); CE(2, 3);
    CE(4, 5); CE(6, 7); CE(2, 4); CE(3, 5); CE(1, 4); CE(3, 6); CE(1, 2); CE(3, 4); CE(5, 6);
  }
  if constexpr (N == 9) {
    CE(0, 3); CE(1, 7); CE(2, 5); CE(4, 8); CE(0, 7); CE(2, 4); CE(3, 8); CE(5, 6); CE(0, 2);
    CE(1, 3); CE(4, 5); CE(7, 8); CE(1, 4); CE(3, 6); CE(5, 7); CE(0, 1); CE(2, 4); CE(3, 5);
    CE(6, 8); CE(2, 3); CE(4, 5); CE(6, 7); CE(1, 2); CE(3, 4); CE(5, 6);
  }
#undef CE
  return v[N / 2];
}

template <int N>
__device__ __forceinline__ uint64_t select_other_network(uint64_t (&v)[N]) {
#define CE(i, j) ce_desc(v[i], v[j])
  if constexpr (N == 3) { CE(0, 1); }
  if constexpr (N == 4) { CE(0, 2); CE(0, 1); CE(1, 2); }
  if constexpr (N == 5) { CE(0, 2); CE(1, 3); CE(0, 1); CE(2, 3); CE(1, 2); }
  if constexpr (N == 6) {
    CE(0, 3); CE(1, 4); CE(0, 2); CE(1, 3); CE(0, 1); CE(2, 4); CE(1, 2); CE(3, 4); CE(2, 3);
  }
  if constexpr (N == 7) {
    CE(0, 5); CE(1, 3); CE(2, 4); CE(1, 2); CE(3, 4); CE(0, 3); CE(2, 5); CE(0, 1); CE(2, 3); CE(1, 2);
  }
  if constexpr (N == 8) {
    CE(0, 6); CE(2, 3); CE(4, 5); CE(0, 2); CE(1, 4); CE(3, 6); CE(0, 1);
    CE(2, 5); CE(3, 4); CE(1, 2); CE(4, 6); CE(2, 3); CE(4, 5); CE(3, 4);
  }
  if constexpr (N == 9) {
    CE(0, 2); CE(1, 3); CE(4, 6); CE(5, 7); CE(0, 4); CE(1, 5); CE(2, 6); CE(3, 7); CE(0, 1);
    CE(2, 3); CE(4, 5); CE(6, 7); CE(2, 4); CE(3, 5); CE(1, 4); CE(3, 6); CE(3, 4);
  }
#undef CE
  return v[N / 2 - 1];
}

template <int N>
__device__ __forceinline__ uint64_t select_quorum_oddeven(uint64_t (&v)[N]) {
#pragma unroll
  for (int r = 0; r < N; ++r) {
#pragma unroll
    for (int i = (r & 1); i + 1 < N; i += 2) ce_desc(v[i], v[i + 1]);
  }
  return v[N / 2];
}

template <bool GATED>
__device__ __forceinline__ uint64_t maybe_commit(uint64_t mci, uint64_t committed, uint64_t first_idx) {
  bool adv = mci > committed;
  if constexpr (GATED) adv = adv && (first_idx != 0) && (mci >= first_idx);
  return adv ? mci : committed;
}

__device__ __forceinline__ uint64_t bytes_equal(uint64_t v, uint64_t pattern) {
  const uint64_t k7f = 0x7f7f7f7f7f7f7f7full;
  const uint64_t x = v ^ pattern;
  uint64_t y = (x & k7f) + k7f;
  y = ~(y | x | k7f);
  return y >> 7;
}

__host__ __device__ constexpr int vote_word_bytes(int n_peers) { return n_peers <= 8 ? 2 : 4; }
typedef unsigned int u32x4p __attribute__((ext_vector_type(4)));

template <int N>
__device__ __forceinline__ uint32_t poll_word(uint32_t w) {
  constexpr uint32_t kLow = 0x55555555u & ((N >= 16) ? 0xffffffffu : ((1u << (2 * N)) - 1u));
  constexpr uint32_t q = N / 2 + 1;
  const uint32_t granted = __popc(w & ~(w >> 1) & kLow);
  const uint32_t rejected = __popc((w >> 1) & ~w & kLow);
  const uint32_t won = granted >= q ? 1u : 0u;
  const uint32_t lost = (won == 0u && rejected >= q) ? 2u : 0u;
  return won | lost;
}

template <typename T>
__device__ __forceinline__ T ld_stream(const T* p) {
  return __builtin_nontemporal_load(p);
}
template <typename T>
__device__ __forceinline__ void st_stream(T* p, T v) {
  __builtin_nontemporal_store(v, p);
}

#define RAFTQ_GLOBAL __attribute__((address_space(1)))
template <bool NT, typename T>
__device__ __forceinline__ T ldg(const T* p) {
  const RAFTQ_GLOBAL T* g = (const RAFTQ_GLOBAL T*)p;
  if constexpr (NT) return __builtin_nontemporal_load(g);
  else return *g;
}
template <bool NT, typename T>
__device__ __forceinline__ void stg(T* p, T v) {
  RAFTQ_GLOBAL T* g = (RAFTQ_GLOBAL T*)p;
  if constexpr (NT) __builtin_nontemporal_store(v, g);
  else *g = v;
}
typedef unsigned int u32x4 __attribute__((ext_vector_type(4)));
__device__ __forceinline__ void stg_u4(uint4* p, uint4 v) {
  u32x4 t;
  t.x = v.x; t.y = v.y; t.z = v.z; t.w = v.w;
  *(RAFTQ_GLOBAL u32x4*)p = t;
}

__device__ __forceinline__ uint32_t wave_sum_u32(uint32_t x) {
#pragma unroll
  for (int o = 32; o > 0; o >>= 1) x += __shfl_xor(x, o, 64);
  return x;
}

constexpr int kLdNT = 1, kStNT = 2, kNoStore = 4;
constexpr int kNoCompute = 8;

template <int N, int GPL, bool COMMIT, bool GATED, bool VOTES>
struct TileRegs {
  static constexpr int kRounds = GPL / 2;
  u64x2 m[COMMIT ? kRounds : 1][N];
  u64x2 c[COMMIT ? kRounds : 1];
  u64x2 f[COMMIT && GATED ? kRounds : 1];
  u32x4p vw[VOTES ? (N <= 8 ? 1 : 2) : 1];
  uint32_t skip = 0;
};

constexpr int kBodyAll = 0, kBodySkip = 1, kBodyNarrow = 2;
constexpr uint32_t kSkipNarrow = 0x100u;

template <int N, bool COMMIT>
__device__ __forceinline__ uint32_t self_max_skip(const SweepArgs& a) {
  if constexpr (!COMMIT || N < 2) {
    return 0;
  } else {
    if (a.self_max == nullptr) return 0;
    const uint32_t w = __builtin_amdgcn_readfirstlane(ldg<false>(a.self_max));
    return (w & kSelfMaxValid) != 0 ? (w & 0xffu) + 1 : 0;
  }
}

template <int N, bool COMMIT>
__device__ __forceinline__ uint32_t tile_body(const SweepArgs& a) {
  const uint32_t skip = self_max_skip<N, COMMIT>(a);
  if constexpr (!COMMIT || N < 3) {
    return skip;
  } else {
    if (N < 5 && skip != 0) return skip;
    if (a.narrow == nullptr) return skip;
    const uint32_t w = __builtin_amdgcn_readfirstlane(ldg<false>(a.narrow));
    return w == kNarrowValid ? kSkipNarrow : skip;
  }
}

template <int N, int GPL, bool COMMIT, bool GATED, bool VOTES, int POLICY, int BLOCK = kBlock, int BODY = kBodyAll>
__device__ __forceinline__ void tile_load(TileRegs<N, GPL, COMMIT, GATED, VOTES>& r, const SweepArgs& a,
                                          const uint32_t tile) {
  constexpr bool NT = (POLICY & kLdNT) != 0;
  constexpr int kTile = BLOCK * GPL;
  constexpr int kRounds = GPL / 2;
  constexpr bool SKIP = BODY == kBodySkip;
  constexpr int kRows = SKIP && N >= 2 ? N - 1 : N;
  static_assert(BODY != kBodyNarrow || N >= 3, "the narrow body is chosen from N = 3 (tile_body)");
  const uint32_t tid = threadIdx.x;
  const uint64_t tile0 = (uint64_t)tile * kTile;
  constexpr int kVoteLanes = kTile / 8;
  if constexpr (VOTES) {
    if (tid < kVoteLanes) {
      const uint8_t* src = a.votes + (tile0 + 8ull * tid) * vote_word_bytes(N);
      r.vw[0] = ldg<NT>(reinterpret_cast<const u32x4p*>(src));
      if constexpr (N > 8) r.vw[1] = ldg<NT>(reinterpret_cast<const u32x4p*>(src + 16));
    }
  }
  if constexpr (COMMIT) {
    const uint64_t* row[kRows];
#pragma unroll
    for (int p = 0; p < kRows; ++p) {
      const uint32_t slot = SKIP ? (uint32_t)p + ((uint32_t)p + 1 >= r.skip ? 1u : 0u) : (uint32_t)p;
      row[p] = a.match + (uint64_t)slot * a.ld;
    }
#pragma unroll
    for (int j = 0; j < kRounds; ++j) {
      const uint64_t g = tile0 + (uint64_t)(tid >> 6) * (64 * GPL) + (uint64_t)j * 128 + 2 * (tid & 63);
      if constexpr (BODY == kBodyNarrow) {
#pragma unroll
        for (int p = 0; p < N; ++p) {
          const uint64_t w = ldg<NT>(reinterpret_cast<const uint64_t*>(a.moff + (uint64_t)p * a.ld + g));
          if (p & 1) r.m[j][p >> 1].y = w;
          else r.m[j][p >> 1].x = w;
        }
        r.m[j][N - 1] = ldg<NT>(reinterpret_cast<const u64x2*>(a.anchor + g));
      } else {
#pragma unroll
        for (int p = 0; p < kRows; ++p) {
          r.m[j][p] = ldg<NT>(reinterpret_cast<const u64x2*>(row[p] + g));
        }
      }
      r.c[j] = ldg<NT>(reinterpret_cast<const u64x2*>(a.committed + g));
      if constexpr (GATED) r.f[j] = ldg<NT>(reinterpret_cast<const u64x2*>(a.first_idx + g));
    }
  }
}

template <int N, bool SKIP>
__device__ __forceinline__ uint64_t quorum_select(uint64_t (&v)[N]) {
  if constexpr (N == 1) return v[0];
  else if constexpr (SKIP) return select_other_network<N>(v);
  else return select_quorum_network<N>(v);
}

template <int N, int BODY, bool XOR, typename Regs>
__device__ __forceinline__ void tile_mci(const Regs& r, const int j, uint64_t& mci0, uint64_t& mci1) {
  if constexpr (BODY == kBodyNarrow) {
    uint32_t v0[N], v1[N];
#pragma unroll
    for (int p = 0; p < N; ++p) {
      const uint64_t w = (p & 1) ? r.m[j][p >> 1].y : r.m[j][p >> 1].x;
      v0[p] = (uint32_t)w;
      v1[p] = (uint32_t)(w >> 32);
    }
    uint32_t s0, s1;
    if constexpr (XOR) {
      s0 = v0[0];
      s1 = v1[0];
#pragma unroll
      for (int p = 1; p < N; ++p) {
        s0 ^= v0[p];
        s1 ^= v1[p];
      }
    } else {
      s0 = select_quorum_network<N, uint32_t>(v0);
      s1 = select_quorum_network<N, uint32_t>(v1);
    }
    mci0 = r.m[j][N - 1].x + s0;
    mci1 = r.m[j][N - 1].y + s1;
  } else {
    constexpr bool SKIP = BODY == kBodySkip;
    constexpr int kRows = SKIP && N >= 2 ? N - 1 : N;
    uint64_t v0[N], v1[N];
#pragma unroll
    for (int p = 0; p < kRows; ++p) {
      v0[p] = r.m[j][p].x;
      v1[p] = r.m[j][p].y;
    }
    if constexpr (XOR) {
      mci0 = v0[0];
      mci1 = v1[0];
#pragma unroll
      for (int p = 1; p < kRows; ++p) {
        mci0 ^= v0[p];
        mci1 ^= v1[p];
      }
    } else {
      mci0 = quorum_select<N, SKIP>(v0);
      mci1 = quorum_select<N, SKIP>(v1);
    }
  }
}

template <int N, int GPL, bool COMMIT, bool GATED, bool VOTES, int POLICY, bool BITS, int BLOCK = kBlock, int BODY = kBodyAll>
__device__ __forceinline__ void tile_finish(const TileRegs<N, GPL, COMMIT, GATED, VOTES>& r, const SweepArgs& a,
                                            const uint32_t tile) {
  constexpr bool STNT = (POLICY & kStNT) != 0;
  constexpr bool NOSTORE = (POLICY & kNoStore) != 0;
  constexpr int kTile = BLOCK * GPL;
  constexpr int kWavesB = BLOCK / 64;
  constexpr int kRounds = GPL / 2;
  const uint32_t tid = threadIdx.x;
  const uint64_t tile0 = (uint64_t)tile * kTile;
  uint32_t n_changed = 0;
  uint32_t won_lost = 0;
  constexpr int kVoteLanes = kTile / 8;
  const bool vote_lane = VOTES && tid < kVoteLanes;

  if constexpr (COMMIT) {
#pragma unroll
    for (int j = 0; j < kRounds; ++j) {
      const uint64_t g = tile0 + (uint64_t)(tid >> 6) * (64 * GPL) + (uint64_t)j * 128 + 2 * (tid & 63);
      uint64_t mci0, mci1;
      tile_mci<N, BODY, (POLICY & kNoCompute) != 0>(r, j, mci0, mci1);
      u64x2 o;
      if constexpr ((POLICY & kNoCompute) != 0) {
        o.x = mci0 ^ r.c[j].x;
        o.y = mci1 ^ r.c[j].y;
      } else {
        o.x = maybe_commit<GATED>(mci0, r.c[j].x, GATED ? r.f[j].x : 0);
        o.y = maybe_commit<GATED>(mci1, r.c[j].y, GATED ? r.f[j].y : 0);
      }
      const bool ch0 = o.x != r.c[j].x;
      const bool ch1 = o.y != r.c[j].y;
      const uint64_t b0 = __ballot(ch0);
      const uint64_t b1 = __ballot(ch1);
      n_changed += __popcll(b0) + __popcll(b1);
      if constexpr (BITS) {
        if (a.changed_bits != nullptr && (tid & 63) == 0) {
          u64x2 w;
          w.x = b0;
          w.y = b1;
          stg<false>(reinterpret_cast<u64x2*>(a.changed_bits + (g >> 6)), w);
        }
      }
      if constexpr (NOSTORE) {
        asm volatile("" ::"v"(o.x), "v"(o.y));
      } else {
        stg<STNT>(reinterpret_cast<u64x2*>(a.committed_out + g), o);
      }
    }
  }

  if constexpr (VOTES) {
    if (vote_lane) {
      const uint64_t g = tile0 + 8ull * tid;
      uint32_t out = 0, n_won = 0, n_lost = 0;
#pragma unroll
      for (int k = 0; k < 8; ++k) {
        uint32_t w;
        if constexpr (N <= 8) {
          const uint32_t pair = k < 2 ? r.vw[0].x : k < 4 ? r.vw[0].y : k < 6 ? r.vw[0].z : r.vw[0].w;
          w = (k & 1) ? pair >> 16 : pair & 0xffffu;
        } else {
          w = k == 0 ? r.vw[0].x : k == 1 ? r.vw[0].y : k == 2 ? r.vw[0].z : k == 3 ? r.vw[0].w
            : k == 4 ? r.vw[1].x : k == 5 ? r.vw[1].y : k == 6 ? r.vw[1].z : r.vw[1].w;
        }
        const uint32_t oc = poll_word<N>(w);
        out |= oc << (2 * k);
        n_won += oc & 1u;
        n_lost += oc >> 1;
      }
      uint16_t* dst = reinterpret_cast<uint16_t*>(a.outcome + (g >> 2));
      if constexpr (NOSTORE) {
        asm volatile("" ::"v"(out));
      } else {
        stg<STNT>(dst, (uint16_t)out);
      }
      won_lost = n_won | (n_lost << 16);
    }
  }

  const uint32_t wl = VOTES ? wave_sum_u32(won_lost) : 0u;
  if ((tid & 63) == 0) {
    uint4 t;
    t.x = n_changed;
    t.y = wl & 0xffffu;
    t.z = wl >> 16;
    t.w = 0;
    stg_u4(a.partials + ((uint64_t)tile * kWavesB + (tid >> 6)), t);
  }
}

template <int N, int GPL, bool COMMIT, bool GATED, bool VOTES, int POLICY, bool BITS, int BLOCK = kBlock>
__device__ __forceinline__ void sweep_tile(const SweepArgs& a, const uint32_t tile) {
  TileRegs<N, GPL, COMMIT, GATED, VOTES> r;
  r.skip = tile_body<N, COMMIT>(a);
  if constexpr (COMMIT && N >= 3) {
    if (r.skip == kSkipNarrow) {
      tile_load<N, GPL, COMMIT, GATED, VOTES, POLICY, BLOCK, kBodyNarrow>(r, a, tile);
      tile_finish<N, GPL, COMMIT, GATED, VOTES, POLICY, BITS, BLOCK, kBodyNarrow>(r, a, tile);
      return;
    }
  }
  if (r.skip != 0) {
    tile_load<N, GPL, COMMIT, GATED, VOTES, POLICY, BLOCK, kBodySkip>(r, a, tile);
    tile_finish<N, GPL, COMMIT, GATED, VOTES, POLICY, BITS, BLOCK, kBodySkip>(r, a, tile);
  } else {
    tile_load<N, GPL, COMMIT, GATED, VOTES, POLICY, BLOCK>(r, a, tile);
    tile_finish<N, GPL, COMMIT, GATED, VOTES, POLICY, BITS, BLOCK>(r, a, tile);
  }
}

template <int N, int GPL, bool COMMIT, bool GATED, bool VOTES, int POLICY, bool BITS, int BLOCK = kBlock>
static __global__ __launch_bounds__(BLOCK) void sweep_kernel(SweepArgs a) {
  sweep_tile<N, GPL, COMMIT, GATED, VOTES, POLICY, BITS, BLOCK>(a, blockIdx.x);
}

template <int N, int GPL, bool COMMIT, bool GATED, bool VOTES, int POLICY, bool BITS, int BLOCK = kBlock>
static __global__ __launch_bounds__(BLOCK) void sweep_set_kernel(const SweepArgs* __restrict__ tab, uint32_t want_bits) {
  SweepArgs a = tab[blockIdx.y];
  if (!want_bits) a.changed_bits = nullptr;
  sweep_tile<N, GPL, COMMIT, GATED, VOTES, POLICY, BITS, BLOCK>(a, blockIdx.x);
}

template <int N, int GPL, bool COMMIT, bool GATED, bool VOTES, int POLICY, bool BITS, int MINW = 1>
static __global__ __launch_bounds__(kBlock, MINW) void sweep_persist_kernel(const SweepArgs* __restrict__ tab,
                                                                      uint32_t tiles_per_member, uint32_t total_tiles,
                                                                      uint32_t want_bits) {
  using Regs = TileRegs<N, GPL, COMMIT, GATED, VOTES>;
  const uint32_t stride = gridDim.x;
  uint32_t t = blockIdx.x;
  if (t >= total_tiles) return;
  auto locate = [&](uint32_t lin, SweepArgs& a, uint32_t& tile) {
    const uint32_t m = lin / tiles_per_member;
    tile = lin - m * tiles_per_member;
    a = tab[m];
    if (!want_bits) a.changed_bits = nullptr;
  };
  auto load = [&](Regs& r, const SweepArgs& a, uint32_t tile) {
    r.skip = tile_body<N, COMMIT>(a);
    if constexpr (COMMIT && N >= 3) {
      if (r.skip == kSkipNarrow) {
        tile_load<N, GPL, COMMIT, GATED, VOTES, POLICY, kBlock, kBodyNarrow>(r, a, tile);
        return;
      }
    }
    if (r.skip != 0) tile_load<N, GPL, COMMIT, GATED, VOTES, POLICY, kBlock, kBodySkip>(r, a, tile);
    else tile_load<N, GPL, COMMIT, GATED, VOTES, POLICY>(r, a, tile);
  };
  auto finish = [&](const Regs& r, const SweepArgs& a, uint32_t tile) {
    if constexpr (COMMIT && N >= 3) {
      if (r.skip == kSkipNarrow) {
        tile_finish<N, GPL, COMMIT, GATED, VOTES, POLICY, BITS, kBlock, kBodyNarrow>(r, a, tile);
        return;
      }
    }
    if (r.skip != 0) tile_finish<N, GPL, COMMIT, GATED, VOTES, POLICY, BITS, kBlock, kBodySkip>(r, a, tile);
    else tile_finish<N, GPL, COMMIT, GATED, VOTES, POLICY, BITS>(r, a, tile);
  };
  Regs A, B;
  SweepArgs aA, aB;
  uint32_t tileA, tileB;
  locate(t, aA, tileA);
  load(A, aA, tileA);
  while (true) {
    t += stride;
    if (t >= total_tiles) {
      finish(A, aA, tileA);
      break;
    }
    locate(t, aB, tileB);
    load(B, aB, tileB);
    finish(A, aA, tileA);
    t += stride;
    if (t >= total_tiles) {
      finish(B, aB, tileB);
      break;
    }
    locate(t, aA, tileA);
    load(A, aA, tileA);
    finish(B, aB, tileB);
  }
}

static __global__ __launch_bounds__(kBlock) void set_counts_kernel(const SweepArgs* __restrict__ tab,
                                                                    const uint64_t* __restrict__ n_partials_of,
                                                                    uint64_t* __restrict__ out) {
  __shared__ uint64_t red[3][kWaves];
  const uint4* p = tab[blockIdx.x].partials;
  const uint64_t n_partials = n_partials_of[blockIdx.x];
  uint64_t c = 0, w = 0, l = 0;
  for (uint64_t i = threadIdx.x; i < n_partials; i += kBlock) {
    const uint4 v = p[i];
    c += v.x;
    w += v.y;
    l += v.z;
  }
#pragma unroll
  for (int o = 32; o > 0; o >>= 1) {
    c += __shfl_xor(c, o, 64);
    w += __shfl_xor(w, o, 64);
    l += __shfl_xor(l, o, 64);
  }
  if ((threadIdx.x & 63) == 0) {
    red[0][threadIdx.x >> 6] = c;
    red[1][threadIdx.x >> 6] = w;
    red[2][threadIdx.x >> 6] = l;
  }
  __syncthreads();
  if (threadIdx.x < 3) {
    uint64_t t = 0;
    for (int k = 0; k < kWaves; ++k) t += red[threadIdx.x][k];
    out[(uint64_t)blockIdx.x * 4 + threadIdx.x] = t;
  }
  if (threadIdx.x == 3) out[(uint64_t)blockIdx.x * 4 + 3] = 0;
}

typedef __attribute__((address_space(3))) void lds_void_t;
typedef const __attribute__((address_space(1))) void global_cvoid_t;

template <int N, int GPL, bool GATED, bool VOTES, bool BITS>
static __global__ __launch_bounds__(kBlock) void sweep_lds_kernel(SweepArgs a) {
  constexpr int kTile = kBlock * GPL;
  constexpr int kRounds = GPL / 2;
  constexpr int kRows = N + 1 + (GATED ? 1 : 0);
  constexpr int kRowBytes = 64 * 16;
  extern __shared__ __attribute__((aligned(16))) unsigned char smem[];
  const uint32_t tid = threadIdx.x;
  const uint32_t lane = tid & 63;
  const uint32_t wave = tid >> 6;
  unsigned char* wbase = smem + (size_t)wave * (kRounds * kRows * kRowBytes);
  const uint64_t tile0 = (uint64_t)blockIdx.x * kTile;
  uint32_t n_changed = 0;
// ... 54 lines not shown
    constexpr int kVoteLanes = kTile / 8;
    if (tid < kVoteLanes) {
      const uint64_t g = tile0 + 8ull * tid;
      const uint8_t* src = a.votes + g * vote_word_bytes(N);
      uint32_t words[8];
      if constexpr (N <= 8) {
        const u32x4p v = *reinterpret_cast<const u32x4p*>(src);
        const uint32_t pr[4] = {v.x, v.y, v.z, v.w};
#pragma unroll
        for (int k = 0; k < 8; ++k) words[k] = (k & 1) ? pr[k >> 1] >> 16 : pr[k >> 1] & 0xffffu;
      } else {
        const u32x4p v0 = *reinterpret_cast<const u32x4p*>(src), v1 = *reinterpret_cast<const u32x4p*>(src + 16);
        words[0] = v0.x; words[1] = v0.y; words[2] = v0.z; words[3] = v0.w;
        words[4] = v1.x; words[5] = v1.y; words[6] = v1.z; words[7] = v1.w;
      }
      uint32_t out = 0, n_won = 0, n_lost = 0;
#pragma unroll
      for (int k = 0; k < 8; ++k) {
        const uint32_t oc = poll_word<N>(words[k]);
        out |= oc << (2 * k);
        n_won += oc & 1u;
        n_lost += oc >> 1;
      }
      *reinterpret_cast<uint16_t*>(a.outcome + (g >> 2)) = (uint16_t)out;
      won_lost = n_won | (n_lost << 16);
    }
  }
  const uint32_t wl = VOTES ? wave_sum_u32(won_lost) : 0u;
  if (lane == 0) {
    uint4 r;
    r.x = n_changed;
    r.y = wl & 0xffffu;
    r.z = wl >> 16;
    r.w = 0;
    a.partials[(uint64_t)blockIdx.x * kWaves + wave] = r;
  }
}

struct DeltaRec {
  uint64_t group, match;
  uint32_t peer, pad;
};
struct Delta16Rec {
  uint64_t match;
  uint32_t group, peer;
};
struct VoteDeltaRec {
  uint64_t group;
  uint32_t peer;
  uint8_t vote, pad[3];
};

constexpr unsigned long long kNoEpoch = ~0ull;
__device__ __forceinline__ bool batch_is_bad(const unsigned long long* bad, unsigned long long epoch_match,
                                             unsigned long long epoch_votes) {
  return bad[0] == epoch_match || bad[1] == epoch_votes;
}

static __global__ __launch_bounds__(kBlock) void self_max_check_kernel(const uint64_t* __restrict__ match, uint64_t ld,
                                                                       uint64_t n_groups, uint32_t n_peers, uint32_t slot,
                                                                       uint32_t* word) {
  bool broken = false;
  for (uint64_t g = (uint64_t)blockIdx.x * kBlock + threadIdx.x; g < n_groups; g += (uint64_t)gridDim.x * kBlock) {
    const uint64_t own = match[(uint64_t)slot * ld + g];
    for (uint32_t p = 0; p < n_peers; ++p) broken |= match[(uint64_t)p * ld + g] > own;
  }
  if (__ballot(broken) != 0 && (threadIdx.x & 63) == 0) *word = 0u;
}

__device__ __forceinline__ bool breaks_self_max(uint32_t w, const uint64_t* match, uint64_t ld, uint64_t group, uint32_t peer,
                                                uint64_t value) {
  if ((w & kSelfMaxValid) == 0) return false;
  const uint32_t slot = w & 0xffu;
  return peer != slot && value > match[(uint64_t)slot * ld + group];
}
__device__ __forceinline__ void clear_self_max_if(bool broken, uint32_t* word) {
  const uint64_t b = __ballot(broken);
  if (b != 0 && (threadIdx.x & 63) == (uint32_t)(__ffsll((unsigned long long)b) - 1)) *word = 0u;
}

static __global__ __launch_bounds__(kBlock) void narrow_build_kernel(const uint64_t* __restrict__ match, uint64_t ld,
                                                                     uint64_t n_groups, uint32_t n_peers,
                                                                     uint64_t* __restrict__ anchor, uint32_t* __restrict__ moff,
                                                                     uint32_t* word) {
  bool broken = false;
  for (uint64_t g = (uint64_t)blockIdx.x * kBlock + threadIdx.x; g < n_groups; g += (uint64_t)gridDim.x * kBlock) {
    uint64_t lo = match[g], hi = lo;
    for (uint32_t p = 1; p < n_peers; ++p) {
      const uint64_t v = match[(uint64_t)p * ld + g];
      lo = v < lo ? v : lo;
      hi = v > hi ? v : hi;
    }
    anchor[g] = lo;
    if (hi - lo > 0xffffffffull) {
      broken = true;
    } else {
      for (uint32_t p = 0; p < n_peers; ++p) moff[(uint64_t)p * ld + g] = (uint32_t)(match[(uint64_t)p * ld + g] - lo);
    }
  }
  if (__ballot(broken) != 0 && (threadIdx.x & 63) == 0) *word = 0u;
}

struct NarrowMirror {
  uint32_t* word;
  const uint64_t* anchor;
  uint32_t* moff;
};
__device__ __forceinline__ bool narrow_follow(uint32_t w, const NarrowMirror& m, uint64_t ld, uint64_t group, uint32_t peer,
                                              uint64_t value) {
  if (w != kNarrowValid) return false;
  const uint64_t base = m.anchor[group];
  if (value < base) return false;
  if (value - base > 0xffffffffull) return true;
  atomicMax(m.moff + (uint64_t)peer * ld + group, (uint32_t)(value - base));
  return false;
}
__device__ __forceinline__ void clear_narrow_if(bool broken, uint32_t* word) { clear_self_max_if(broken, word); }

template <typename Rec>
static __global__ __launch_bounds__(kBlock) void deltas_in_kernel(const Rec* __restrict__ src, Rec* __restrict__ dst,
                                                                  uint64_t n, uint64_t n_groups, uint32_t n_peers,
                                                                  unsigned long long* bad_epoch, uint64_t* bad_host,
                                                                  unsigned long long epoch) {
  const uint64_t i = (uint64_t)blockIdx.x * kBlock + threadIdx.x;
  bool bad = false;
  if (i < n) {
    const Rec r = src[i];
    dst[i] = r;
    bad = r.group >= n_groups || r.peer >= n_peers;
  }
  if (__ballot(bad) != 0 && (threadIdx.x & 63) == 0) {
    atomicMax(bad_epoch, epoch);
    *bad_host = epoch;
  }
}

template <typename Rec>
static __global__ __launch_bounds__(kBlock) void deltas_in_apply_kernel(const Rec* __restrict__ src, uint64_t n, uint64_t* match,
                                                                        uint64_t ld, uint64_t n_groups, uint32_t n_peers,
                                                                        unsigned long long* bad_epoch, uint64_t* bad_host,
                                                                        unsigned long long epoch, uint32_t* self_max,
                                                                        NarrowMirror mirror) {
  const uint64_t i = (uint64_t)blockIdx.x * kBlock + threadIdx.x;
  const uint32_t w = *self_max;
  const uint32_t nw = *mirror.word;
  bool bad = false, broken = false, wide = false;
  if (i < n) {
    const Rec r = src[i];
    bad = r.group >= n_groups || r.peer >= n_peers;
    if (!bad) {
      broken = breaks_self_max(w, match, ld, r.group, r.peer, r.match);
      wide = narrow_follow(nw, mirror, ld, r.group, r.peer, r.match);
      atomicMax(reinterpret_cast<unsigned long long*>(match + (uint64_t)r.peer * ld + r.group), (unsigned long long)r.match);
    }
  }
  clear_self_max_if(broken, self_max);
  clear_narrow_if(wide, mirror.word);
  if (__ballot(bad) != 0 && (threadIdx.x & 63) == 0) {
    atomicMax(bad_epoch, epoch);
    *bad_host = epoch;
  }
}

template <typename Rec>
static __global__ __launch_bounds__(kBlock) void apply_deltas_kernel(uint64_t* match, uint64_t ld,
                                                              const Rec* __restrict__ d, uint64_t n,
                                                              const unsigned long long* bad,
                                                              unsigned long long epoch_match, unsigned long long epoch_votes,
                                                              uint32_t* self_max, NarrowMirror mirror) {
  if (batch_is_bad(bad, epoch_match, epoch_votes)) return;
  const uint64_t i = (uint64_t)blockIdx.x * kBlock + threadIdx.x;
  const uint32_t w = *self_max;
  const uint32_t nw = *mirror.word;
  bool broken = false, wide = false;
  if (i < n) {
    const Rec r = d[i];
    broken = breaks_self_max(w, match, ld, r.group, r.peer, r.match);
    wide = narrow_follow(nw, mirror, ld, r.group, r.peer, r.match);
    atomicMax(reinterpret_cast<unsigned long long*>(match + (uint64_t)r.peer * ld + r.group),
              (unsigned long long)r.match);
  }
  clear_self_max_if(broken, self_max);
  clear_narrow_if(wide, mirror.word);
}

struct TermDeltaRec {
  uint64_t group, cur_term, first_idx_cur_term;
};
static __global__ __launch_bounds__(kBlock) void apply_term_deltas_kernel(uint64_t* first_idx,
                                                                   const TermDeltaRec* __restrict__ d, uint64_t n) {
  const uint64_t i = (uint64_t)blockIdx.x * kBlock + threadIdx.x;
  if (i >= n) return;
  const TermDeltaRec r = d[i];
  first_idx[r.group] = r.cur_term == 0 ? 0ull : r.first_idx_cur_term;
}

static __global__ __launch_bounds__(kBlock) void vote_deltas_in_kernel(const VoteDeltaRec* __restrict__ src,
                                                                       VoteDeltaRec* __restrict__ dst, uint64_t n,
                                                                       uint64_t n_groups, uint32_t n_peers,
                                                                       unsigned long long* bad_epoch, uint64_t* bad_host,
                                                                       unsigned long long epoch) {
  const uint64_t i = (uint64_t)blockIdx.x * kBlock + threadIdx.x;
  bool bad = false;
  if (i < n) {
    const VoteDeltaRec r = src[i];
    dst[i] = r;
    bad = r.group >= n_groups || r.peer >= n_peers || (unsigned)(r.vote - 1) > 1u;
  }
  if (__ballot(bad) != 0 && (threadIdx.x & 63) == 0) {
    atomicMax(bad_epoch, epoch);
    *bad_host = epoch;
  }
}

__device__ __forceinline__ bool vote_rec_ok(const VoteDeltaRec& r, uint64_t n_groups, uint32_t n_peers) {
  return r.group < n_groups && r.peer < n_peers && (unsigned)(r.vote - 1) <= 1u;
}

static __global__ __launch_bounds__(kBlock) void vote_claim_kernel(uint32_t* claim, uint64_t ld,
                                                            const VoteDeltaRec* __restrict__ d, uint64_t n,
                                                            const unsigned long long* bad, unsigned long long epoch_match,
                                                            unsigned long long epoch_votes, uint64_t n_groups,
                                                            uint32_t n_peers, int each) {
  if (!each && batch_is_bad(bad, epoch_match, epoch_votes)) return;
  const uint64_t i = (uint64_t)blockIdx.x * kBlock + threadIdx.x;
  if (i >= n) return;
  const VoteDeltaRec r = d[i];
  if (each && !vote_rec_ok(r, n_groups, n_peers)) return;
  atomicMin(claim + (uint64_t)r.peer * ld + r.group, (uint32_t)i);
}

static __global__ __launch_bounds__(kBlock) void vote_apply_kernel(uint8_t* votes, int wide, uint32_t* claim, uint64_t ld,
                                                            const VoteDeltaRec* __restrict__ d, uint64_t n,
                                                            const unsigned long long* bad, unsigned long long epoch_match,
                                                            unsigned long long epoch_votes, uint64_t n_groups,
                                                            uint32_t n_peers, int each) {
  if (!each && batch_is_bad(bad, epoch_match, epoch_votes)) return;
  const uint64_t i = (uint64_t)blockIdx.x * kBlock + threadIdx.x;
  if (i >= n) return;
  const VoteDeltaRec r = d[i];
  if (each && !vote_rec_ok(r, n_groups, n_peers)) return;
  const uint64_t slot = (uint64_t)r.peer * ld + r.group;
  if (claim[slot] != (uint32_t)i) return;
  unsigned int* word = reinterpret_cast<unsigned int*>(votes) + (wide ? r.group : r.group >> 1);
  const unsigned sh = (wide ? 0u : (unsigned)(r.group & 1ull) * 16u) + 2u * r.peer;
  const unsigned nv = (unsigned)r.vote << sh;
  unsigned old = *word;
  while (true) {
    const unsigned cur = (old >> sh) & 3u;
    if (cur == 1u || cur == 2u) break;
    const unsigned seen = atomicCAS(word, old, (old & ~(3u << sh)) | nv);
    if (seen == old) break;
    old = seen;
  }
  claim[slot] = 0xffffffffu;
}

struct Advance {
  uint64_t group, old_commit, new_commit;
};
struct Advance16 {
  uint64_t new_commit;
  uint32_t group, advanced_by;
};
__device__ __forceinline__ Advance make_advance(Advance*, uint64_t g, uint64_t o, uint64_t n) { return Advance{g, o, n}; }
__device__ __forceinline__ Advance16 make_advance(Advance16*, uint64_t g, uint64_t o, uint64_t n) {
  const uint64_t by = n - o;
  return Advance16{n, (uint32_t)g, by > 0xfffffffeull ? 0xffffffffu : (uint32_t)by};
}

static __global__ __launch_bounds__(1024) void scan_partials_kernel(const uint4* __restrict__ partials, uint64_t n_waves,
                                                             uint64_t* __restrict__ offsets, uint64_t* total, int field) {
  __shared__ uint64_t wave_tot[16];
  const uint32_t tid = threadIdx.x, lane = tid & 63, w = tid >> 6;
  const uint64_t per = (n_waves + 1023) / 1024;
  const uint64_t lo = (uint64_t)tid * per, hi = lo + per < n_waves ? lo + per : n_waves;
  const uint32_t* p32 = reinterpret_cast<const uint32_t*>(partials) + field;
// ... 30 lines not shown
    for (uint64_t i = lo; i < hi; ++i) {
      offsets[i] = run;
      run += p32[i * 4];
    }
  }
  if (tid == 1023) *total = pre + incl;
}

template <int GPL, typename Adv>
static __global__ __launch_bounds__(kBlock) void compact_changed_kernel(const uint64_t* changed_bits,
                                                                 const uint4* __restrict__ partials,
                                                                 const uint64_t* old_commit,
                                                                 const uint64_t* new_commit,
                                                                 Adv* out, uint64_t cap, uint64_t* total,
                                                                 const uint64_t* __restrict__ wave_offsets) {
  constexpr int kTile = kBlock * GPL;
  constexpr int kRounds = GPL / 2;
  __shared__ uint64_t red[kWaves];
  __shared__ uint32_t mine[kWaves];
  const uint32_t tid = threadIdx.x, lane = tid & 63, wave = tid >> 6;
  const uint64_t first_wave = (uint64_t)blockIdx.x * kWaves;
  const uint32_t* cnt = reinterpret_cast<const uint32_t*>(partials);
  uint64_t acc = 0;
  if (wave_offsets == nullptr) {
    uint32_t a0 = 0, a1 = 0, a2 = 0, a3 = 0;
    uint64_t i = tid;
    for (; i + 3 * kBlock < first_wave; i += 4 * kBlock) {
      a0 += cnt[4 * i];
      a1 += cnt[4 * (i + kBlock)];
      a2 += cnt[4 * (i + 2 * kBlock)];
      a3 += cnt[4 * (i + 3 * kBlock)];
    }
    for (; i < first_wave; i += kBlock) a0 += cnt[4 * i];
    acc = (uint64_t)a0 + a1 + a2 + a3;
#pragma unroll
    for (int o = 32; o > 0; o >>= 1) acc += __shfl_xor(acc, o, 64);
  } else if (lane == 0 && wave == 0) {
    acc = wave_offsets[first_wave];
  }
  if (lane == 0) red[wave] = acc;
  if (tid < kWaves) mine[tid] = cnt[4 * (first_wave + tid)];
  __syncthreads();
  uint64_t pos = 0;
#pragma unroll
  for (int k = 0; k < kWaves; ++k) pos += red[k];
  if (blockIdx.x == gridDim.x - 1 && tid == 0) {
    uint64_t t = pos;
    for (int k = 0; k < kWaves; ++k) t += mine[k];
    *total = t;
  }
  for (uint32_t k = 0; k < wave; ++k) pos += mine[k];
  const uint64_t below = lane == 0 ? 0ull : (~0ull >> (64 - lane));
#pragma unroll
  for (int j = 0; j < kRounds; ++j) {
    const uint64_t g0 = (uint64_t)blockIdx.x * kTile + (uint64_t)wave * (64 * GPL) + (uint64_t)j * 128;
    const uint64_t b0 = changed_bits[(g0 >> 6)];
    const uint64_t b1 = changed_bits[(g0 >> 6) + 1];
    const bool e = (b0 >> lane) & 1, o = (b1 >> lane) & 1;
    const uint64_t rank = __popcll(b0 & below) + __popcll(b1 & below);
    if (e) {
      const uint64_t g = g0 + 2 * lane, s = pos + rank;
      if (s < cap) out[s] = make_advance((Adv*)nullptr, g, old_commit[g], new_commit[g]);
    }
    if (o) {
      const uint64_t g = g0 + 2 * lane + 1, s = pos + rank + (e ? 1 : 0);
      if (s < cap) out[s] = make_advance((Adv*)nullptr, g, old_commit[g], new_commit[g]);
    }
    pos += __popcll(b0) + __popcll(b1);
  }
}

static __global__ void raise_flag_kernel(uint64_t* flag, uint64_t epoch) {
  if (threadIdx.x == 0 && blockIdx.x == 0) __hip_atomic_store(flag, epoch, __ATOMIC_RELAXED, __HIP_MEMORY_SCOPE_SYSTEM);
}

template <int N, int GPL, bool GATED, int POLICY>
static __global__ __launch_bounds__(kBlock) void sweep_segments_kernel(SweepArgs a, Advance16* list, unsigned int* counts_host, unsigned int* counts_dev) {
  constexpr bool STNT = (POLICY & kStNT) != 0;
  constexpr int kTile = kBlock * GPL;
  constexpr int kRounds = GPL / 2;
  __shared__ uint32_t wave_cnt[kWaves];
  const uint32_t tid = threadIdx.x, lane = tid & 63, wave = tid >> 6, tile = blockIdx.x;
  TileRegs<N, GPL, true, GATED, false> r;
  r.skip = tile_body<N, true>(a);
  const bool narrow = N >= 3 && r.skip == kSkipNarrow;
  if (narrow) {
    if constexpr (N >= 3) tile_load<N, GPL, true, GATED, false, POLICY, kBlock, kBodyNarrow>(r, a, tile);
  } else if (r.skip != 0) {
    tile_load<N, GPL, true, GATED, false, POLICY, kBlock, kBodySkip>(r, a, tile);
  } else {
    tile_load<N, GPL, true, GATED, false, POLICY>(r, a, tile);
  }
  const uint64_t tile0 = (uint64_t)tile * kTile;
  u64x2 nw[kRounds];
  uint64_t even[kRounds], odd[kRounds];
  uint32_t n_changed = 0;
#pragma unroll
  for (int j = 0; j < kRounds; ++j) {
    const uint64_t g = tile0 + (uint64_t)wave * (64 * GPL) + (uint64_t)j * 128 + 2 * lane;
    uint64_t mci0 = 0, mci1 = 0;
    if (narrow) {
      if constexpr (N >= 3) tile_mci<N, kBodyNarrow, false>(r, j, mci0, mci1);
    } else if (r.skip != 0) {
      tile_mci<N, kBodySkip, false>(r, j, mci0, mci1);
    } else {
      tile_mci<N, kBodyAll, false>(r, j, mci0, mci1);
    }
    u64x2 o;
    o.x = maybe_commit<GATED>(mci0, r.c[j].x, GATED ? r.f[j].x : 0);
    o.y = maybe_commit<GATED>(mci1, r.c[j].y, GATED ? r.f[j].y : 0);
    even[j] = __ballot(o.x != r.c[j].x);
    odd[j] = __ballot(o.y != r.c[j].y);
    n_changed += __popcll(even[j]) + __popcll(odd[j]);
    nw[j] = o;
    if (a.changed_bits != nullptr && lane == 0) {
      u64x2 w;
      w.x = even[j];
      w.y = odd[j];
      stg<false>(reinterpret_cast<u64x2*>(a.changed_bits + (g >> 6)), w);
    }
    stg<STNT>(reinterpret_cast<u64x2*>(a.committed_out + g), o);
  }
  if (lane == 0) {
    uint4 t;
    t.x = n_changed;
    t.y = t.z = t.w = 0;
    stg_u4(a.partials + ((uint64_t)tile * kWaves + wave), t);
    wave_cnt[wave] = n_changed;
  }
  __syncthreads();
  uint64_t pos = tile0;
  for (uint32_t k = 0; k < wave; ++k) pos += wave_cnt[k];
  if (tid == 0) {
    uint32_t tile_cnt = 0;
#pragma unroll
    for (int k = 0; k < kWaves; ++k) tile_cnt += wave_cnt[k];
    counts_host[tile] = tile_cnt;
    counts_dev[tile] = tile_cnt;
  }
  const uint64_t below = lane == 0 ? 0ull : (~0ull >> (64 - lane));
#pragma unroll
  for (int j = 0; j < kRounds; ++j) {
    const uint64_t g0 = tile0 + (uint64_t)wave * (64 * GPL) + (uint64_t)j * 128;
    const bool e = (even[j] >> lane) & 1, o = (odd[j] >> lane) & 1;
    const uint64_t rank = __popcll(even[j] & below) + __popcll(odd[j] & below);
    if (e) list[pos + rank] = make_advance((Advance16*)nullptr, g0 + 2 * lane, r.c[j].x, nw[j].x);
    if (o) list[pos + rank + (e ? 1 : 0)] = make_advance((Advance16*)nullptr, g0 + 2 * lane + 1, r.c[j].y, nw[j].y);
    pos += __popcll(even[j]) + __popcll(odd[j]);
  }
}

static __global__ __launch_bounds__(kBlock) void raise_flag_segments_kernel(uint64_t* flag, uint32_t epoch, const unsigned int* counts_dev, uint32_t n_tiles) {
  __shared__ uint32_t red[kWaves];
  uint32_t acc = 0;
  for (uint32_t i = threadIdx.x; i < n_tiles; i += kBlock) acc += counts_dev[i];
#pragma unroll
  for (int o = 32; o > 0; o >>= 1) acc += __shfl_xor(acc, o, 64);
  if ((threadIdx.x & 63) == 0) red[threadIdx.x >> 6] = acc;
  __syncthreads();
  if (threadIdx.x == 0) {
    uint32_t total = 0;
#pragma unroll
    for (int k = 0; k < kWaves; ++k) total += red[k];
    __hip_atomic_store(flag, ((uint64_t)epoch << 32) | total, __ATOMIC_RELAXED, __HIP_MEMORY_SCOPE_SYSTEM);
  }
}

struct VoterSweepArgs {
  SweepArgs s;
  const uint16_t* voters;
};

__device__ __forceinline__ uint64_t sel_u64(bool c, uint64_t a, uint64_t b) { return c ? a : b; }

template <int N, int... I>
__device__ __forceinline__ uint64_t pick_sorted(const uint64_t (&v)[N], uint32_t idx, std::integer_sequence<int, I...>) {
  uint64_t r = v[0];
  ((r = sel_u64(idx == (uint32_t)(I + 1), v[I + 1], r)), ...);
  return r;
}
template <int N, int... I>
__device__ __forceinline__ void zero_non_voters(uint64_t (&v)[N], uint32_t mask, std::integer_sequence<int, I...>) {
  ((v[I] = sel_u64(((mask >> I) & 1u) != 0, v[I], 0ull)), ...);
}

template <int N>
__device__ __forceinline__ uint64_t select_quorum_voters(uint64_t (&v)[N], uint32_t mask) {
  zero_non_voters<N>(v, mask, std::make_integer_sequence<int, N>{});
  if constexpr (N >= 2) (void)select_quorum_network<N>(v);
  return pick_sorted<N>(v, (uint32_t)__popc(mask) >> 1, std::make_integer_sequence<int, N - 1>{});
}

__device__ __forceinline__ uint32_t spread_even(uint32_t m) {
// ... 620 lines not shown
```

raftsql_amd/csrc/raftq_step_kernels.hpp:

```cpp
#pragma once
#include <hip/hip_runtime.h>
#include <stdint.h>

#include "raftq_kernels.hpp"

namespace raftqk {

struct MsgRec {
  uint64_t group, term, log_term, index, commit, reject_hint;
  uint32_t from;
  uint8_t type, reject, pad[2];
  uint64_t resv;
};
struct StepOutRec {
  uint64_t group, term, index, log_term, commit, last_index;
  uint32_t to, vote, lead;
  uint8_t type, reject, flags, role;
};
struct LogDeltaRec {
  uint64_t group, last_index, last_term, commit_to;
};
struct StepOutC {
  uint64_t term, index, commit, aux;
  uint8_t vote, lead, type, reject, flags, role, pad[2];
// ... 130 lines not shown
  if (fl & kMsgfHold) return kTake;
  const uint8_t t = m.type;
  const bool local = t == kMsgHup || t == kMsgBeat;
  const bool known = local || t == kMsgApp || t == kMsgAppResp || t == kMsgVote || t == kMsgVoteResp ||
                     t == kMsgHeartbeat || t == kMsgHeartbeatResp;
  if (!known || (!local && m.from >= n_peers)) return kBad;
  if (recs == kRecsWire && ((m.pad[1] & 1u) != 0 || m.pad[0] >= n_peers)) return kBad;
  return kTake;
}
__device__ __forceinline__ void put_skipped(void* out, uint64_t i, uint8_t compact) {
  StepOutRec o;
  __builtin_memset(&o, 0, sizeof o);
  o.type = kOutSkipped;
  put_result(out, i, o, compact);
}

static __global__ __launch_bounds__(kBlock) void step_keys_kernel(const MsgRec* __restrict__ msgs,
                                                                  uint64_t* __restrict__ keys,
                                                                  uint32_t* __restrict__ order, uint64_t n,
                                                                  uint64_t n_groups, uint32_t n_peers,
                                                                  unsigned int* bad, bool msg_flags, uint8_t recs,
                                                                  void* __restrict__ out, uint8_t compact) {
  const uint64_t i = (uint64_t)blockIdx.x * kBlock + threadIdx.x;
  bool is_bad = false;
  if (i < n) {
    const RecClass c = classify(msgs[i], n_groups, n_peers, msg_flags, recs);
    is_bad = c == kBad;
    keys[i] = c == kTake ? msgs[i].group : c == kSkip ? n_groups : 0;
    order[i] = (uint32_t)i;
    if (c == kSkip) put_skipped(out, i, compact);
  }
  if (__ballot(is_bad) != 0 && (threadIdx.x & 63) == 0) atomicOr(bad, 1u);
}

constexpr uint32_t kMaxRun = 32;
constexpr uint32_t kNil = 0xffffffffu;

template <bool MASKED>
struct NodeT {
  const NodeArrays& a;
  uint64_t g;
  uint64_t term, last_index, last_term, committed, first_idx;
  uint64_t mt[kMaxPeers];
  uint32_t mt_dirty = 0;
  uint32_t vote, lead;
  uint32_t vw = 0;
  uint32_t lst_head, lst_cnt, lst_min;
  uint8_t role;
  bool held = false;
  bool at_tail = false, host_owns = false;
  uint64_t committed0, first_idx0;
  uint8_t role0;
  bool vw_known = false, vw_dirty = false, elapsed_reset = false;
  uint32_t vmask = 0;

  __device__ NodeT(const NodeArrays& arr, uint64_t group, const uint16_t* voters = nullptr) : a(arr), g(group) {
    if constexpr (MASKED) vmask = voters[g];
    const NodeRec r = a.rec[g];
    term = r.term; last_index = r.last_index; last_term = r.last_term;
    vote = r.vote; lead = r.lead;
    lst_head = r.lst_head; lst_cnt = r.lst_cnt; lst_min = r.lst_min;
    committed = committed0 = r.committed;
    first_idx = first_idx0 = r.first_idx;
    role = role0 = r.role;
#pragma unroll
    for (int p = 0; p < kMaxPeers; ++p) mt[p] = r.match[p];
    if (a.at_tail != nullptr) at_tail = ((a.at_tail[g >> 6] >> (g & 63)) & 1ull) != 0;
  }
  __device__ void store(bool list_reset = true) const {
    NodeRec r;
    r.term = term; r.last_index = last_index; r.last_term = last_term;
    r.vote = (uint8_t)vote; r.lead = (uint8_t)lead;
    r.role = role; r.pad = 0;
    r.lst_head = list_reset ? kNil : lst_head;
    r.lst_cnt = list_reset ? 0u : lst_cnt;
    r.lst_min = list_reset ? kNil : lst_min;
    r.committed = committed;
    r.first_idx = first_idx;
#pragma unroll
    for (int p = 0; p < kMaxPeers; ++p) r.match[p] = mt[p];
    a.rec[g] = r;
    if (committed != committed0) a.committed[g] = committed;
    if (role != role0) a.role[g] = role;
    if (first_idx != first_idx0) a.first_idx[g] = first_idx;
#pragma unroll
    for (int p = 0; p < kMaxPeers; ++p)
      if ((mt_dirty >> p) & 1u) a.match[(uint64_t)p * a.ld + g] = mt[p];
    if (mt_dirty != 0 && a.self_max != nullptr) {
      const uint32_t w = *a.self_max;
      if ((w & kSelfMaxValid) != 0) {
        const uint64_t own = match(w & 0xffu);
        bool broken = false;
#pragma unroll
        for (uint32_t p = 0; p < (uint32_t)kMaxPeers; ++p) broken |= p < a.n_peers && mt[p] > own;
        if (broken) *a.self_max = 0u;
      }
    }
    if (mt_dirty != 0 && a.self_max != nullptr && a.self_max[1] != 0u) a.self_max[1] = 0u;
    if (elapsed_reset) a.elapsed[g] = 0;
    if (vw_dirty) {
      if (a.n_peers <= 8) reinterpret_cast<uint16_t*>(a.votes)[g] = (uint16_t)vw;
      else reinterpret_cast<uint32_t*>(a.votes)[g] = vw;
    }
  }
  __device__ void set_first_idx(uint64_t v) { first_idx = v; }
  __device__ uint64_t get_first_idx() const { return first_idx; }
  __device__ void set_votes(uint32_t w) {
    vw = w;
    vw_known = vw_dirty = true;
  }
  __device__ uint32_t get_votes() {
    if (!vw_known) {
      vw = a.n_peers <= 8 ? (uint32_t)reinterpret_cast<const uint16_t*>(a.votes)[g] : reinterpret_cast<const uint32_t*>(a.votes)[g];
      vw_known = true;
    }
    return vw;
  }
  __device__ uint64_t match(uint32_t p) const {
    uint64_t v = 0;
#pragma unroll
    for (uint32_t k = 0; k < (uint32_t)kMaxPeers; ++k) v = k == p ? mt[k] : v;
    return v;
  }
  __device__ void set_match(uint32_t p, uint64_t v) {
#pragma unroll
    for (uint32_t k = 0; k < (uint32_t)kMaxPeers; ++k) mt[k] = k == p ? v : mt[k];
    mt_dirty |= 1u << p;
  }
  __device__ uint32_t quorum() const {
    if constexpr (MASKED) return ((uint32_t)__popc(vmask) >> 1) + 1u;
    else return a.n_peers / 2 + 1;
  }
  __device__ bool counts(uint32_t p, uint32_t n) const {
    if constexpr (MASKED) return ((vmask >> p) & 1u) != 0;
    else return p < n;
  }

  __device__ void reset(uint64_t t) {
    if (term != t) { term = t; vote = 0; }
    lead = 0;
    elapsed_reset = true;
    set_votes(0);
#pragma unroll
    for (uint32_t p = 0; p < (uint32_t)kMaxPeers; ++p)
      if (p < a.n_peers) {
        const uint64_t v = p == a.self ? last_index : 0;
        if (mt[p] != v) mt_dirty |= 1u << p;
        mt[p] = v;
      }
  }
  __device__ void become_follower(uint64_t t, uint32_t new_lead) {
    reset(t);
    lead = new_lead;
    role = kFollower;
    set_first_idx(0);
  }
  __device__ void become_candidate() {
    reset(term + 1);
    vote = a.self + 1;
    role = kCandidate;
    set_first_idx(0);
  }
  __device__ bool maybe_commit() {
    uint64_t m[kMaxPeers];
    const uint32_t n = a.n_peers, q = quorum();
#pragma unroll
    for (uint32_t p = 0; p < kMaxPeers; ++p) m[p] = counts(p, n) ? mt[p] : 0;
// ... 307 lines not shown
```

raftsql_amd/engine.py:

```python
from __future__ import annotations

import ctypes as C
from dataclasses import dataclass
from typing import Optional

import numpy as np

from . import _lib
from ._lib import (SWEEP_CACHED, SWEEP_CHANGED, SWEEP_COMMIT, SWEEP_GATED, SWEEP_LDS, SWEEP_NO_ADOPT,
                   SWEEP_STREAM, SWEEP_VOTES, Advance, Counts, Delta, RaftqError, VoteDelta)

__all__ = ["QuorumEngine", "SweepSet", "sweep_many_async", "SweepCounts", "device_count", "RaftqError", "pinned_empty", "pinned_copy", "SWEEP_COMMIT", "SWEEP_GATED",
           "SWEEP_VOTES", "SWEEP_NO_ADOPT", "SWEEP_LDS", "SWEEP_CHANGED", "SWEEP_STREAM", "SWEEP_CACHED"]


@dataclass
class SweepCounts:
    n_changed: int
    n_won: int
    n_lost: int


def device_count() -> int:
    lib = _lib.load()
# ... 268 lines not shown
        nv = 0 if vote_deltas is None else len(vote_deltas)
        n = C.c_uint64(0)
        self._chk(self._lib.raftq_cycle(
            self._h, _ptr(deltas) if nd else None, nd, _ptr(vote_deltas) if nv else None, nv, flags,
            None, int(cap), C.byref(n), None))
        return int(n.value)

    def cycle(self, flags: int, deltas: Optional[np.ndarray] = None, vote_deltas: Optional[np.ndarray] = None,
              cap: Optional[int] = None, out: Optional[np.ndarray] = None, want_counts: bool = True):
        nd = 0 if deltas is None else len(deltas)
        nv = 0 if vote_deltas is None else len(vote_deltas)
        if nd:
            assert deltas.dtype == self._DELTA_DT and deltas.flags.c_contiguous
        if nv:
            assert vote_deltas.dtype == self._VDELTA_DT and vote_deltas.flags.c_contiguous
        cap = (self.n_groups if cap is None else int(cap))
        if out is None:
            out = np.empty(cap, dtype=self._ADV_DT)
        n = C.c_uint64(0)
        c = Counts()
        self._chk(self._lib.raftq_cycle(
            self._h, _ptr(deltas) if nd else None, nd, _ptr(vote_deltas) if nv else None, nv, flags,
            _ptr(out) if cap else None, cap, C.byref(n), C.byref(c) if want_counts else None))
        total = int(n.value)
        cnt = SweepCounts(int(c.n_changed), int(c.n_won), int(c.n_lost)) if want_counts else None
        return out[: min(total, cap)], total, cnt

    def step_async(self, flags: int) -> None:
        self._chk(self._lib.raftq_step_async(self._h, flags))

    def wait(self, want_counts: bool = False) -> Optional[SweepCounts]:
        if not want_counts:
            self._chk(self._lib.raftq_wait(self._h, None))
            return None
        c = Counts()
        self._chk(self._lib.raftq_wait(self._h, C.byref(c)))
        return SweepCounts(int(c.n_changed), int(c.n_won), int(c.n_lost))

    def sweep(self, flags: int) -> SweepCounts:
        self.step_async(flags)
        return self.wait(want_counts=True)

    def commit_advance(self, gated: bool = False):
        out = np.empty(self.n_groups, dtype=np.uint64)
        n = C.c_uint64(0)
        self._chk(self._lib.raftq_commit_advance(self._h, int(gated), _ptr(out), C.byref(n)))
        return out, int(n.value)

    def vote_tally(self):
        out = np.empty(self.n_groups, dtype=np.uint8)
        c = Counts()
        self._chk(self._lib.raftq_vote_tally(self._h, _ptr(out), C.byref(c)))
        return out, SweepCounts(int(c.n_changed), int(c.n_won), int(c.n_lost))

    def read_committed(self) -> np.ndarray:
        out = np.empty(self.n_groups, dtype=np.uint64)
        self._chk(self._lib.raftq_read_committed(self._h, _ptr(out)))
        return out

    def read_outcome(self) -> np.ndarray:
        out = np.empty(self.n_groups, dtype=np.uint8)
        self._chk(self._lib.raftq_read_outcome(self._h, _ptr(out)))
        return out

    def read_match(self) -> np.ndarray:
        out = np.empty((self.n_peers, self.n_groups), dtype=np.uint64)
        self._chk(self._lib.raftq_read_match(self._h, _ptr(out)))
        return out

    def self_max(self) -> int:
        s = C.c_int32(-1)
        self._chk(self._lib.raftq_self_max(self._h, C.byref(s)))
        return int(s.value)

    def narrow(self) -> bool:
        v = C.c_int32(0)
        self._chk(self._lib.raftq_narrow(self._h, C.byref(v)))
        return bool(v.value)

    def narrow_rebuild(self) -> bool:
        self._chk(self._lib.raftq_narrow_rebuild(self._h))
        return self.narrow()

    def read_votes(self) -> np.ndarray:
        out = np.empty((self.n_peers, self.n_groups), dtype=np.uint8)
        self._chk(self._lib.raftq_read_votes(self._h, _ptr(out)))
        return out

    def collect_changed(self, cap: Optional[int] = None):
        cap = self.n_groups if cap is None else int(cap)
        arr = (Advance * cap)()
        n = C.c_uint64(0)
        self._chk(self._lib.raftq_collect_changed(self._h, C.addressof(arr) if cap else None, cap, C.byref(n)))
        a = np.frombuffer(arr, dtype=np.dtype([("group", "<u8"), ("old_commit", "<u8"), ("new_commit", "<u8")]))
        return a[: min(int(n.value), cap)].copy(), int(n.value)

    def set_timers(self, election_tick: int = 10, heartbeat_tick: int = 1, seed: int = 0x1000) -> None:
        self._chk(self._lib.raftq_set_timers(self._h, election_tick, heartbeat_tick, seed))

    def load_roles(self, role: np.ndarray, elapsed: Optional[np.ndarray] = None) -> None:
        r = np.ascontiguousarray(role, dtype=np.uint8)
        if r.shape != (self.n_groups,):
            raise ValueError("role must be [G]")
        e = None if elapsed is None else np.ascontiguousarray(elapsed, dtype=np.uint32)
        self._chk(self._lib.raftq_load_roles(self._h, _ptr(r), _ptr(e) if e is not None else None))

    def tick(self, want_counts: bool = True):
        if not want_counts:
            self._chk(self._lib.raftq_tick(self._h, None))
            return None
        c = _lib.TickCounts()
        self._chk(self._lib.raftq_tick(self._h, C.byref(c)))
        return int(c.n_hup), int(c.n_beat)

    def read_tick(self):
        a = np.empty(self.n_groups, dtype=np.uint8)
        e = np.empty(self.n_groups, dtype=np.uint32)
        r = np.empty(self.n_groups, dtype=np.uint8)
        self._chk(self._lib.raftq_read_tick(self._h, _ptr(a), _ptr(e), _ptr(r)))
        return a, e, r

    def collect_hups(self, cap: Optional[int] = None):
        cap = self.n_groups if cap is None else int(cap)
        out = np.empty(cap, dtype=np.uint64)
        n = C.c_uint64(0)
        self._chk(self._lib.raftq_collect_hups(self._h, _ptr(out) if cap else None, cap, C.byref(n)))
        return out[: min(cap, int(n.value))], int(n.value)

    def collect_beats(self, cap: Optional[int] = None):
        cap = self.n_groups if cap is None else int(cap)
        out = np.empty(cap, dtype=np.uint64)
        n = C.c_uint64(0)
        self._chk(self._lib.raftq_collect_beats(self._h, _ptr(out) if cap else None, cap, C.byref(n)))
        return out[: min(cap, int(n.value))], int(n.value)

    def tick_collect(self, hup_cap: Optional[int] = None, beat_cap: Optional[int] = None):
        hc = self.n_groups if hup_cap is None else int(hup_cap)
        bc = self.n_groups if beat_cap is None else int(beat_cap)
        hups, beats = np.empty(hc, dtype=np.uint64), np.empty(bc, dtype=np.uint64)
        nh, nb = C.c_uint64(0), C.c_uint64(0)
        self._chk(self._lib.raftq_tick_collect(self._h, _ptr(hups) if hc else None, hc, C.byref(nh), _ptr(beats) if bc else None, bc,
                                               C.byref(nb)))
        return hups[: min(hc, int(nh.value))], int(nh.value), beats[: min(bc, int(nb.value))], int(nb.value)

    def tick_collect_lists(self, hup_cap: Optional[int] = None, beat_cap: Optional[int] = None, beat_bitmap: bool = False):
        hc = self.n_groups if hup_cap is None else int(hup_cap)
        bc = self.n_groups if beat_cap is None else int(beat_cap)
        nh, nb = C.c_uint64(0), C.c_uint64(0)
        self._chk(self._lib.raftq_tick_collect_lists(self._h, _lib.TICK_BEAT_BITMAP if beat_bitmap else 0, hc, bc, C.byref(nh), C.byref(nb)))
        ph, pb, pm = C.c_void_p(None), C.c_void_p(None), C.c_void_p(None)
        lh, lb, lm = C.c_uint64(0), C.c_uint64(0), C.c_uint64(0)
        self._chk(self._lib.raftq_last_tick_lists(self._h, C.byref(ph), C.byref(lh), C.byref(pb), C.byref(lb), C.byref(pm), C.byref(lm)))

        def view(p, n, dt):
            if not n:
                return np.empty(0, dtype=dt)
            return np.frombuffer((C.c_char * (int(n) * np.dtype(dt).itemsize)).from_address(p.value), dtype=dt)

        hups = view(ph, lh.value, np.uint32)
        second = view(pm, lm.value, np.uint64) if beat_bitmap else view(pb, lb.value, np.uint32)
        return hups, int(nh.value), second, int(nb.value)

    def campaign(self, groups, self_peer: int = 0) -> None:
        g = np.ascontiguousarray(groups, dtype=np.uint64)
        self._chk(self._lib.raftq_campaign(self._h, _ptr(g) if len(g) else None, len(g), self_peer))

# ... 93 lines not shown
```

Baseline: 129.7 billion.

## Store narrowed 32-bit gate offsets so gated narrow sweeps skip 64-bit first_idx loads

Adds an extra 32-bit row to the narrow offset table that holds each group's first_idx relative to its anchor, plus a validity word. When both the narrow and the gate word are valid, the gated commit sweep reads this compact row (two groups per 64-bit load) in place of the 64-bit first_idx array and compares in 32-bit space. This cuts per-group memory traffic on the gated commit path. In exchange, term updates, narrow rebuilds, clones and step kernels must keep the gate row in sync or invalidate it, and the sweep gains another body variant and two extra branches.

```diff
diff --git a/go/raftq/engine_more.go b/go/raftq/engine_more.go
--- a/go/raftq/engine_more.go
+++ b/go/raftq/engine_more.go
@@ -28,6 +28,14 @@
 }
 
 func (e *Engine) NarrowRebuild() error { return e.err(C.raftq_narrow_rebuild(e.h)) }
+
+func (e *Engine) GateNarrow() (bool, error) {
+	var valid C.int32_t
+	if err := e.err(C.raftq_gate_narrow(e.h, &valid)); err != nil {
+		return false, err
+	}
+	return valid != 0, nil
+}
 
 func (e *Engine) SetStream(stream unsafe.Pointer) error { return e.err(C.raftq_set_stream(e.h, stream)) }
 func (e *Engine) Stream() unsafe.Pointer                { return C.raftq_get_stream(e.h) }
diff --git a/include/raftq.h b/include/raftq.h
--- a/include/raftq.h
+++ b/include/raftq.h
@@ -122,6 +122,7 @@
 int raftq_self_max(raftq_t* h, int32_t* slot_out);
 int raftq_narrow(raftq_t* h, int32_t* valid_out);
 int raftq_narrow_rebuild(raftq_t* h);
+int raftq_gate_narrow(raftq_t* h, int32_t* valid_out);
 int raftq_read_votes(raftq_t* h, uint8_t* votes_out );
 int raftq_collect_changed(raftq_t* h, raftq_advance_t* out, uint64_t cap, uint64_t* n);
 
diff --git a/raftsql_amd/_lib.py b/raftsql_amd/_lib.py
--- a/raftsql_amd/_lib.py
+++ b/raftsql_amd/_lib.py
@@ -80,6 +80,7 @@
     ("raftq_self_max", C.c_int, [_H, C.POINTER(C.c_int32)]),
     ("raftq_narrow", C.c_int, [_H, C.POINTER(C.c_int32)]),
     ("raftq_narrow_rebuild", C.c_int, [_H]),
+    ("raftq_gate_narrow", C.c_int, [_H, C.POINTER(C.c_int32)]),
     ("raftq_read_votes", C.c_int, [_H, C.c_void_p]),
     ("raftq_collect_changed", C.c_int, [_H, C.c_void_p, C.c_uint64, C.POINTER(C.c_uint64)]),
     ("raftq_set_timers", C.c_int, [_H, C.c_uint32, C.c_uint32, C.c_uint64]),
diff --git a/raftsql_amd/csrc/raftq_capi.hip b/raftsql_amd/csrc/raftq_capi.hip
--- a/raftsql_amd/csrc/raftq_capi.hip
+++ b/raftsql_amd/csrc/raftq_capi.hip
@@ -240,19 +240,56 @@
     return RAFTQ_OK;
   }
   if (!h->anchor) {
+    const bool gate = h->have_terms && !h->gate_off;
+    const size_t rows = (size_t)h->N + (gate ? 1 : 0);
     const hipError_t e = raftq_buf::alloc_group({{(void**)&h->anchor, h->ld * sizeof(uint64_t)},
-                                                 {(void**)&h->moff, (size_t)h->N * h->ld * sizeof(uint32_t)}},
+                                                 {(void**)&h->moff, rows * h->ld * sizeof(uint32_t)}},
                                                 h->stream);
     if (e != hipSuccess) {
       (void)hipGetLastError();
       return RAFTQ_OK;
     }
+    h->gate_row = gate;
     if (h->in_set) h->in_set->tab_stale = true;
+  } else if (h->have_terms) {
+    if (int rc = raftq_detail::ensure_gate_row(h)) return rc;
   }
   HIPCHK(h, hipMemsetD32Async((hipDeviceptr_t)h->narrow_word(), (int)kNarrowValid, 1, h->stream));
+  HIPCHK(h, hipMemsetD32Async((hipDeviceptr_t)h->gate_word(), (int)(h->goff() ? kGateValid : 0u), 1, h->stream));
   const uint64_t blocks = std::min<uint64_t>((h->G + kBlock - 1) / kBlock, 4096);
   hipLaunchKernelGGL(narrow_build_kernel, dim3((unsigned)std::max<uint64_t>(blocks, 1)), dim3(kBlock), 0, h->stream,
-                     (const uint64_t*)h->match, h->ld, h->G, h->N, h->anchor, h->moff, h->narrow_word());
+                     (const uint64_t*)h->match, h->ld, h->G, h->N, h->anchor, h->moff, h->narrow_word(),
+                     (const uint64_t*)h->first_idx, h->goff());
+  HIPCHK(h, hipGetLastError());
+  return RAFTQ_OK;
+}
+int raftq_detail::ensure_gate_row(raftq_t* h) {
+  if (!h->anchor || h->gate_row || h->narrow_off || h->gate_off) return RAFTQ_OK;
+  uint32_t* grown = nullptr;
+  const size_t row = h->ld * sizeof(uint32_t);
+  if (raftq_buf::alloc_group({{(void**)&grown, ((size_t)h->N + 1) * row}}, h->stream) != hipSuccess) {
+    (void)hipGetLastError();
+    return RAFTQ_OK;
+  }
+  const hipError_t e = hipMemcpyAsync(grown, h->moff, (size_t)h->N * row, hipMemcpyDeviceToDevice, h->stream);
+  const hipError_t e2 = e == hipSuccess ? hipStreamSynchronize(h->stream) : e;
+  if (e2 != hipSuccess) {
+    raftq_buf::free_device(grown);
+    HIPCHK(h, e2);
+  }
+  raftq_buf::free_device(h->moff);
+  h->moff = grown;
+  h->gate_row = true;
+  if (h->in_set) h->in_set->tab_stale = true;
+  return RAFTQ_OK;
+}
+int raftq_detail::gate_build(raftq_t* h) {
+  if (int rc = raftq_detail::ensure_gate_row(h)) return rc;
+  if (!h->goff()) return RAFTQ_OK;
+  HIPCHK(h, hipMemsetD32Async((hipDeviceptr_t)h->gate_word(), (int)kGateValid, 1, h->stream));
+  const uint64_t blocks = std::min<uint64_t>((h->G + kBlock - 1) / kBlock, 4096);
+  hipLaunchKernelGGL(gate_build_kernel, dim3((unsigned)std::max<uint64_t>(blocks, 1)), dim3(kBlock), 0, h->stream,
+                     (const uint64_t*)h->first_idx, (const uint64_t*)h->anchor, h->G, h->goff(), h->gate_word());
   HIPCHK(h, hipGetLastError());
   return RAFTQ_OK;
 }
@@ -368,6 +405,8 @@
     {
       const char* nr = std::getenv("RAFTQ_NARROW");
       h->narrow_off = nr && std::strcmp(nr, "0") == 0;
+      const char* gn = std::getenv("RAFTQ_GATE_NARROW");
+      h->gate_off = gn && std::strcmp(gn, "0") == 0;
     }
     e = hipMemsetD32Async((hipDeviceptr_t)h->self_max, (int)(kSelfMaxValid | 0u), 1, h->stream);
     if (e != hipSuccess) { rc = fail(h, RAFTQ_EHIP, std::string("hipMemsetD32Async: ") + hipGetErrorString(e)); break; }
@@ -471,8 +510,9 @@
     if (cur_term[g] == 0) f[g] = 0;
   HIPCHK(h, hipMemcpyAsync(h->first_idx, f.data(), h->G * 8, hipMemcpyHostToDevice, h->stream));
   dense_changed(h);
-  HIPCHK(h, hipStreamSynchronize(h->stream));
   h->have_terms = true;
+  if (int rc = raftq_detail::gate_build(h)) return rc;
+  HIPCHK(h, hipStreamSynchronize(h->stream));
   return RAFTQ_OK;
 }
 
@@ -607,7 +647,7 @@
   const dim3 grid((unsigned)((m + kBlock - 1) / kBlock));
   dense_changed(h);
   hipLaunchKernelGGL(apply_term_deltas_kernel, grid, dim3(kBlock), 0, h->stream, h->first_idx,
-                     (const TermDeltaRec*)h->stage.d, m);
+                     (const TermDeltaRec*)h->stage.d, m, h->gate_word(), (const uint64_t*)h->anchor, h->goff());
   HIPCHK(h, hipGetLastError());
   HIPCHK(h, hipStreamSynchronize(h->stream));
   h->have_terms = true;
@@ -908,6 +948,16 @@
   HIPCHK(h, hipMemcpyAsync(&w, h->narrow_word(), sizeof w, hipMemcpyDeviceToHost, h->stream));
   HIPCHK(h, hipStreamSynchronize(h->stream));
   *valid = w == kNarrowValid ? 1 : 0;
+  return RAFTQ_OK;
+}
+
+int raftq_gate_narrow(raftq_t* h, int32_t* valid) {
+  if (int rc = use_device_idle(h, "raftq_gate_narrow")) return rc;
+  if (!valid) return fail(h, RAFTQ_EINVAL, "raftq_gate_narrow: null argument");
+  uint32_t w = 0;
+  HIPCHK(h, hipMemcpyAsync(&w, h->gate_word(), sizeof w, hipMemcpyDeviceToHost, h->stream));
+  HIPCHK(h, hipStreamSynchronize(h->stream));
+  *valid = w == kGateValid ? 1 : 0;
   return RAFTQ_OK;
 }
 
@@ -1973,11 +2023,16 @@
   HIPCHK(dst, hipMemcpyAsync(dst->self_max, src->self_max, sizeof(uint32_t), hipMemcpyDeviceToDevice, dst->stream));
   if (src->anchor && !dst->narrow_off && !dst->anchor) {
     if (raftq_buf::alloc_group({{(void**)&dst->anchor, ld * sizeof(uint64_t), raftq_buf::Kind::device, nullptr, false},
-                                {(void**)&dst->moff, (size_t)dst->N * ld * sizeof(uint32_t), raftq_buf::Kind::device, nullptr, false}},
+                                {(void**)&dst->moff, ((size_t)dst->N + (src->gate_row && !dst->gate_off ? 1 : 0)) * ld * sizeof(uint32_t), raftq_buf::Kind::device, nullptr, false}},
                                dst->stream) != hipSuccess)
       (void)hipGetLastError();
-    else if (dst->in_set) dst->in_set->tab_stale = true;
-  }
+    else {
+      dst->gate_row = src->gate_row && !dst->gate_off;
+      if (dst->in_set) dst->in_set->tab_stale = true;
+    }
+  }
+  if (src->gate_row)
+    if (int rc = raftq_detail::ensure_gate_row(dst)) return rc;
   if (src->anchor && dst->anchor && !dst->narrow_off) {
     HIPCHK(dst, hipMemcpyAsync(dst->anchor, src->anchor, ld * sizeof(uint64_t), hipMemcpyDeviceToDevice, dst->stream));
     HIPCHK(dst, hipMemcpyAsync(dst->moff, src->moff, (size_t)dst->N * ld * sizeof(uint32_t), hipMemcpyDeviceToDevice, dst->stream));
@@ -1985,6 +2040,12 @@
   } else {
     HIPCHK(dst, hipMemsetAsync(dst->narrow_word(), 0, sizeof(uint32_t), dst->stream));
   }
+  if (src->goff() && dst->goff()) {
+    HIPCHK(dst, hipMemcpyAsync(dst->goff(), src->goff(), ld * sizeof(uint32_t), hipMemcpyDeviceToDevice, dst->stream));
+    HIPCHK(dst, hipMemcpyAsync(dst->gate_word(), src->gate_word(), sizeof(uint32_t), hipMemcpyDeviceToDevice, dst->stream));
+  } else {
+    HIPCHK(dst, hipMemsetAsync(dst->gate_word(), 0, sizeof(uint32_t), dst->stream));
+  }
   if (src->voters) HIPCHK(dst, hipMemcpyAsync(dst->voters, src->voters, ld * sizeof(uint16_t), hipMemcpyDeviceToDevice, dst->stream));
   HIPCHK(dst, hipStreamSynchronize(dst->stream));
   dst->have_terms = src->have_terms;
diff --git a/raftsql_amd/csrc/raftq_internal.hpp b/raftsql_amd/csrc/raftq_internal.hpp
--- a/raftsql_amd/csrc/raftq_internal.hpp
+++ b/raftsql_amd/csrc/raftq_internal.hpp
@@ -55,6 +55,10 @@
   uint32_t* moff = nullptr;
   bool narrow_off = false;
   uint32_t* narrow_word() const { return self_max + 1; }
+  bool gate_row = false;
+  bool gate_off = false;
+  uint32_t* gate_word() const { return self_max + 2; }
+  uint32_t* goff() const { return gate_row ? moff + (size_t)N * ld : nullptr; }
   raftqk::NarrowMirror narrow_mirror() const { return raftqk::NarrowMirror{self_max + 1, anchor, moff}; }
   uint64_t compact_epoch = 0;
   uint64_t compact_epoch_armed = 0;
@@ -213,6 +217,8 @@
 inline bool masked_bcast(const raftq_t* h) { return h->voters != nullptr && h->bcast_voters; }
 int self_max_check(raftq_t* h);
 int narrow_build(raftq_t* h);
+int ensure_gate_row(raftq_t* h);
+int gate_build(raftq_t* h);
 int ensure_staging(raftq_t* h, size_t bytes);
 int ensure_ingest(raftq_t* h, size_t bytes);
 int ensure_tick_state(raftq_t* h);
diff --git a/raftsql_amd/csrc/raftq_kernels.hpp b/raftsql_amd/csrc/raftq_kernels.hpp
--- a/raftsql_amd/csrc/raftq_kernels.hpp
+++ b/raftsql_amd/csrc/raftq_kernels.hpp
@@ -33,6 +33,16 @@
 
 constexpr uint32_t kNarrowValid = 1u;
 
+constexpr uint32_t kGateValid = 1u;
+constexpr uint32_t kGateNever = 0xffffffffu;
+__device__ __forceinline__ bool gate_encode(uint64_t first_idx, uint64_t anchor, uint32_t* out) {
+  if (first_idx == 0) { *out = kGateNever; return true; }
+  if (first_idx <= anchor) { *out = 0u; return true; }
+  const uint64_t d = first_idx - anchor;
+  *out = d >= 0xffffffffull ? kGateNever : (uint32_t)d;
+  return d != 0xffffffffull;
+}
+
 template <typename T>
 __device__ __forceinline__ void ce_desc(T& a, T& b) {
   const bool gt = a > b;
@@ -111,6 +121,11 @@
   bool adv = mci > committed;
   if constexpr (GATED) adv = adv && (first_idx != 0) && (mci >= first_idx);
   return adv ? mci : committed;
+}
+__device__ __forceinline__ uint64_t maybe_commit_narrow(uint64_t anchor, uint32_t s, uint64_t committed, uint32_t goff) {
+  const bool pass = goff != kGateNever && s >= goff;
+  const uint64_t mci = anchor + s;
+  return (mci > committed && pass) ? mci : committed;
 }
 
 __device__ __forceinline__ uint64_t bytes_equal(uint64_t v, uint64_t pattern) {
@@ -183,8 +198,9 @@
   uint32_t skip = 0;
 };
 
-constexpr int kBodyAll = 0, kBodySkip = 1, kBodyNarrow = 2;
-constexpr uint32_t kSkipNarrow = 0x100u;
+constexpr int kBodyAll = 0, kBodySkip = 1, kBodyNarrow = 2, kBodyNarrowGate = 3;
+constexpr uint32_t kSkipNarrow = 0x100u, kSkipNarrowGate = 0x200u;
+constexpr bool body_is_narrow(int body) { return body == kBodyNarrow || body == kBodyNarrowGate; }
 
 template <int N, bool COMMIT>
 __device__ __forceinline__ uint32_t self_max_skip(const SweepArgs& a) {
@@ -197,7 +213,7 @@
   }
 }
 
-template <int N, bool COMMIT>
+template <int N, bool COMMIT, bool GATED = false>
 __device__ __forceinline__ uint32_t tile_body(const SweepArgs& a) {
   const uint32_t skip = self_max_skip<N, COMMIT>(a);
   if constexpr (!COMMIT || N < 3) {
@@ -206,6 +222,10 @@
     if (N < 5 && skip != 0) return skip;
     if (a.narrow == nullptr) return skip;
     const uint32_t w = __builtin_amdgcn_readfirstlane(ldg<false>(a.narrow));
+    if constexpr (GATED) {
+      const uint32_t gw = __builtin_amdgcn_readfirstlane(ldg<false>(a.narrow + 1));
+      if (w == kNarrowValid && gw == kGateValid) return kSkipNarrowGate;
+    }
     return w == kNarrowValid ? kSkipNarrow : skip;
   }
 }
@@ -218,7 +238,8 @@
   constexpr int kRounds = GPL / 2;
   constexpr bool SKIP = BODY == kBodySkip;
   constexpr int kRows = SKIP && N >= 2 ? N - 1 : N;
-  static_assert(BODY != kBodyNarrow || N >= 3, "the narrow body is chosen from N = 3 (tile_body)");
+  static_assert(!body_is_narrow(BODY) || N >= 3, "the narrow body is chosen from N = 3 (tile_body)");
+  static_assert(BODY != kBodyNarrowGate || (COMMIT && GATED), "the narrow gate belongs to a gated commit sweep");
   const uint32_t tid = threadIdx.x;
   const uint64_t tile0 = (uint64_t)tile * kTile;
   constexpr int kVoteLanes = kTile / 8;
@@ -239,7 +260,7 @@
 #pragma unroll
     for (int j = 0; j < kRounds; ++j) {
       const uint64_t g = tile0 + (uint64_t)(tid >> 6) * (64 * GPL) + (uint64_t)j * 128 + 2 * (tid & 63);
-      if constexpr (BODY == kBodyNarrow) {
+      if constexpr (body_is_narrow(BODY)) {
 #pragma unroll
         for (int p = 0; p < N; ++p) {
           const uint64_t w = ldg<NT>(reinterpret_cast<const uint64_t*>(a.moff + (uint64_t)p * a.ld + g));
@@ -254,7 +275,11 @@
         }
       }
       r.c[j] = ldg<NT>(reinterpret_cast<const u64x2*>(a.committed + g));
-      if constexpr (GATED) r.f[j] = ldg<NT>(reinterpret_cast<const u64x2*>(a.first_idx + g));
+      if constexpr (BODY == kBodyNarrowGate) {
+        r.f[j].x = ldg<NT>(reinterpret_cast<const uint64_t*>(a.moff + (uint64_t)N * a.ld + g));
+      } else if constexpr (GATED) {
+        r.f[j] = ldg<NT>(reinterpret_cast<const u64x2*>(a.first_idx + g));
+      }
     }
   }
 }
@@ -266,29 +291,33 @@
   else return select_quorum_network<N>(v);
 }
 
+template <int N, bool XOR, typename Regs>
+__device__ __forceinline__ void tile_sel_narrow(const Regs& r, const int j, uint32_t& s0, uint32_t& s1) {
+  uint32_t v0[N], v1[N];
+#pragma unroll
+  for (int p = 0; p < N; ++p) {
+    const uint64_t w = (p & 1) ? r.m[j][p >> 1].y : r.m[j][p >> 1].x;
+    v0[p] = (uint32_t)w;
+    v1[p] = (uint32_t)(w >> 32);
+  }
+  if constexpr (XOR) {
+    s0 = v0[0];
+    s1 = v1[0];
+#pragma unroll
+    for (int p = 1; p < N; ++p) {
+      s0 ^= v0[p];
+      s1 ^= v1[p];
+    }
+  } else {
+    s0 = select_quorum_network<N, uint32_t>(v0);
+    s1 = select_quorum_network<N, uint32_t>(v1);
+  }
+}
 template <int N, int BODY, bool XOR, typename Regs>
 __device__ __forceinline__ void tile_mci(const Regs& r, const int j, uint64_t& mci0, uint64_t& mci1) {
-  if constexpr (BODY == kBodyNarrow) {
-    uint32_t v0[N], v1[N];
-#pragma unroll
-    for (int p = 0; p < N; ++p) {
-      const uint64_t w = (p & 1) ? r.m[j][p >> 1].y : r.m[j][p >> 1].x;
-      v0[p] = (uint32_t)w;
-      v1[p] = (uint32_t)(w >> 32);
-    }
+  if constexpr (body_is_narrow(BODY)) {
     uint32_t s0, s1;
-    if constexpr (XOR) {
-      s0 = v0[0];
-      s1 = v1[0];
-#pragma unroll
-      for (int p = 1; p < N; ++p) {
-        s0 ^= v0[p];
-        s1 ^= v1[p];
-      }
-    } else {
-      s0 = select_quorum_network<N, uint32_t>(v0);
-      s1 = select_quorum_network<N, uint32_t>(v1);
-    }
+    tile_sel_narrow<N, XOR>(r, j, s0, s1);
     mci0 = r.m[j][N - 1].x + s0;
     mci1 = r.m[j][N - 1].y + s1;
   } else {
@@ -334,13 +363,19 @@
 #pragma unroll
     for (int j = 0; j < kRounds; ++j) {
       const uint64_t g = tile0 + (uint64_t)(tid >> 6) * (64 * GPL) + (uint64_t)j * 128 + 2 * (tid & 63);
-      uint64_t mci0, mci1;
-      tile_mci<N, BODY, (POLICY & kNoCompute) != 0>(r, j, mci0, mci1);
+      [[maybe_unused]] uint64_t mci0, mci1;
       u64x2 o;
-      if constexpr ((POLICY & kNoCompute) != 0) {
+      if constexpr (BODY == kBodyNarrowGate && (POLICY & kNoCompute) == 0) {
+        uint32_t s0, s1;
+        tile_sel_narrow<N, false>(r, j, s0, s1);
+        o.x = maybe_commit_narrow(r.m[j][N - 1].x, s0, r.c[j].x, (uint32_t)r.f[j].x);
+        o.y = maybe_commit_narrow(r.m[j][N - 1].y, s1, r.c[j].y, (uint32_t)(r.f[j].x >> 32));
+      } else if constexpr ((POLICY & kNoCompute) != 0) {
+        tile_mci<N, BODY, true>(r, j, mci0, mci1);
         o.x = mci0 ^ r.c[j].x;
         o.y = mci1 ^ r.c[j].y;
       } else {
+        tile_mci<N, BODY, false>(r, j, mci0, mci1);
         o.x = maybe_commit<GATED>(mci0, r.c[j].x, GATED ? r.f[j].x : 0);
         o.y = maybe_commit<GATED>(mci1, r.c[j].y, GATED ? r.f[j].y : 0);
       }
@@ -408,7 +443,14 @@
 template <int N, int GPL, bool COMMIT, bool GATED, bool VOTES, int POLICY, bool BITS, int BLOCK = kBlock>
 __device__ __forceinline__ void sweep_tile(const SweepArgs& a, const uint32_t tile) {
   TileRegs<N, GPL, COMMIT, GATED, VOTES> r;
-  r.skip = tile_body<N, COMMIT>(a);
+  r.skip = tile_body<N, COMMIT, GATED>(a);
+  if constexpr (COMMIT && GATED && N >= 3) {
+    if (r.skip == kSkipNarrowGate) {
+      tile_load<N, GPL, COMMIT, GATED, VOTES, POLICY, BLOCK, kBodyNarrowGate>(r, a, tile);
+      tile_finish<N, GPL, COMMIT, GATED, VOTES, POLICY, BITS, BLOCK, kBodyNarrowGate>(r, a, tile);
+      return;
+    }
+  }
   if constexpr (COMMIT && N >= 3) {
     if (r.skip == kSkipNarrow) {
       tile_load<N, GPL, COMMIT, GATED, VOTES, POLICY, BLOCK, kBodyNarrow>(r, a, tile);
@@ -452,7 +494,13 @@
     if (!want_bits) a.changed_bits = nullptr;
   };
   auto load = [&](Regs& r, const SweepArgs& a, uint32_t tile) {
-    r.skip = tile_body<N, COMMIT>(a);
+    r.skip = tile_body<N, COMMIT, GATED>(a);
+    if constexpr (COMMIT && GATED && N >= 3) {
+      if (r.skip == kSkipNarrowGate) {
+        tile_load<N, GPL, COMMIT, GATED, VOTES, POLICY, kBlock, kBodyNarrowGate>(r, a, tile);
+        return;
+      }
+    }
     if constexpr (COMMIT && N >= 3) {
       if (r.skip == kSkipNarrow) {
         tile_load<N, GPL, COMMIT, GATED, VOTES, POLICY, kBlock, kBodyNarrow>(r, a, tile);
@@ -463,6 +511,12 @@
     else tile_load<N, GPL, COMMIT, GATED, VOTES, POLICY>(r, a, tile);
   };
   auto finish = [&](const Regs& r, const SweepArgs& a, uint32_t tile) {
+    if constexpr (COMMIT && GATED && N >= 3) {
+      if (r.skip == kSkipNarrowGate) {
+        tile_finish<N, GPL, COMMIT, GATED, VOTES, POLICY, BITS, kBlock, kBodyNarrowGate>(r, a, tile);
+        return;
+      }
+    }
     if constexpr (COMMIT && N >= 3) {
       if (r.skip == kSkipNarrow) {
         tile_finish<N, GPL, COMMIT, GATED, VOTES, POLICY, BITS, kBlock, kBodyNarrow>(r, a, tile);
@@ -683,8 +737,9 @@
 static __global__ __launch_bounds__(kBlock) void narrow_build_kernel(const uint64_t* __restrict__ match, uint64_t ld,
                                                                      uint64_t n_groups, uint32_t n_peers,
                                                                      uint64_t* __restrict__ anchor, uint32_t* __restrict__ moff,
-                                                                     uint32_t* word) {
-  bool broken = false;
+                                                                     uint32_t* word, const uint64_t* __restrict__ first_idx,
+                                                                     uint32_t* __restrict__ goff) {
+  bool broken = false, no_gate = false;
   for (uint64_t g = (uint64_t)blockIdx.x * kBlock + threadIdx.x; g < n_groups; g += (uint64_t)gridDim.x * kBlock) {
     uint64_t lo = match[g], hi = lo;
     for (uint32_t p = 1; p < n_peers; ++p) {
@@ -693,6 +748,11 @@
       hi = v > hi ? v : hi;
     }
     anchor[g] = lo;
+    if (goff != nullptr) {
+      uint32_t d;
+      no_gate |= !gate_encode(first_idx[g], lo, &d);
+      goff[g] = d;
+    }
     if (hi - lo > 0xffffffffull) {
       broken = true;
     } else {
@@ -700,6 +760,18 @@
     }
   }
   if (__ballot(broken) != 0 && (threadIdx.x & 63) == 0) *word = 0u;
+  if (__ballot(no_gate) != 0 && (threadIdx.x & 63) == 0) word[1] = 0u;
+}
+static __global__ __launch_bounds__(kBlock) void gate_build_kernel(const uint64_t* __restrict__ first_idx,
+                                                                   const uint64_t* __restrict__ anchor, uint64_t n_groups,
+                                                                   uint32_t* __restrict__ goff, uint32_t* gate_word) {
+  bool no_gate = false;
+  for (uint64_t g = (uint64_t)blockIdx.x * kBlock + threadIdx.x; g < n_groups; g += (uint64_t)gridDim.x * kBlock) {
+    uint32_t d;
+    no_gate |= !gate_encode(first_idx[g], anchor[g], &d);
+    goff[g] = d;
+  }
+  if (__ballot(no_gate) != 0 && (threadIdx.x & 63) == 0) *gate_word = 0u;
 }
 
 struct NarrowMirror {
@@ -789,11 +861,23 @@
   uint64_t group, cur_term, first_idx_cur_term;
 };
 static __global__ __launch_bounds__(kBlock) void apply_term_deltas_kernel(uint64_t* first_idx,
-                                                                   const TermDeltaRec* __restrict__ d, uint64_t n) {
+                                                                   const TermDeltaRec* __restrict__ d, uint64_t n,
+                                                                   uint32_t* gate_word, const uint64_t* __restrict__ anchor,
+                                                                   uint32_t* goff) {
   const uint64_t i = (uint64_t)blockIdx.x * kBlock + threadIdx.x;
-  if (i >= n) return;
-  const TermDeltaRec r = d[i];
-  first_idx[r.group] = r.cur_term == 0 ? 0ull : r.first_idx_cur_term;
+  const uint32_t gw = goff != nullptr ? *gate_word : 0u;
+  bool no_gate = false;
+  if (i < n) {
+    const TermDeltaRec r = d[i];
+    const uint64_t f = r.cur_term == 0 ? 0ull : r.first_idx_cur_term;
+    first_idx[r.group] = f;
+    if (gw == kGateValid) {
+      uint32_t e;
+      no_gate = !gate_encode(f, anchor[r.group], &e);
+      goff[r.group] = e;
+    }
+  }
+  if (goff != nullptr) clear_self_max_if(no_gate, gate_word);
 }
 
 static __global__ __launch_bounds__(kBlock) void vote_deltas_in_kernel(const VoteDeltaRec* __restrict__ src,
@@ -990,9 +1074,12 @@
   __shared__ uint32_t wave_cnt[kWaves];
   const uint32_t tid = threadIdx.x, lane = tid & 63, wave = tid >> 6, tile = blockIdx.x;
   TileRegs<N, GPL, true, GATED, false> r;
-  r.skip = tile_body<N, true>(a);
+  r.skip = tile_body<N, true, GATED>(a);
   const bool narrow = N >= 3 && r.skip == kSkipNarrow;
-  if (narrow) {
+  const bool narrow_gate = GATED && N >= 3 && r.skip == kSkipNarrowGate;
+  if (narrow_gate) {
+    if constexpr (GATED && N >= 3) tile_load<N, GPL, true, GATED, false, POLICY, kBlock, kBodyNarrowGate>(r, a, tile);
+  } else if (narrow) {
     if constexpr (N >= 3) tile_load<N, GPL, true, GATED, false, POLICY, kBlock, kBodyNarrow>(r, a, tile);
   } else if (r.skip != 0) {
     tile_load<N, GPL, true, GATED, false, POLICY, kBlock, kBodySkip>(r, a, tile);
@@ -1007,16 +1094,25 @@
   for (int j = 0; j < kRounds; ++j) {
     const uint64_t g = tile0 + (uint64_t)wave * (64 * GPL) + (uint64_t)j * 128 + 2 * lane;
     uint64_t mci0 = 0, mci1 = 0;
-    if (narrow) {
-      if constexpr (N >= 3) tile_mci<N, kBodyNarrow, false>(r, j, mci0, mci1);
-    } else if (r.skip != 0) {
-      tile_mci<N, kBodySkip, false>(r, j, mci0, mci1);
+    u64x2 o;
+    if (narrow_gate) {
+      if constexpr (GATED && N >= 3) {
+        uint32_t s0, s1;
+        tile_sel_narrow<N, false>(r, j, s0, s1);
+        o.x = maybe_commit_narrow(r.m[j][N - 1].x, s0, r.c[j].x, (uint32_t)r.f[j].x);
+        o.y = maybe_commit_narrow(r.m[j][N - 1].y, s1, r.c[j].y, (uint32_t)(r.f[j].x >> 32));
+      }
     } else {
-      tile_mci<N, kBodyAll, false>(r, j, mci0, mci1);
-    }
-    u64x2 o;
-    o.x = maybe_commit<GATED>(mci0, r.c[j].x, GATED ? r.f[j].x : 0);
-    o.y = maybe_commit<GATED>(mci1, r.c[j].y, GATED ? r.f[j].y : 0);
+      if (narrow) {
+        if constexpr (N >= 3) tile_mci<N, kBodyNarrow, false>(r, j, mci0, mci1);
+      } else if (r.skip != 0) {
+        tile_mci<N, kBodySkip, false>(r, j, mci0, mci1);
+      } else {
+        tile_mci<N, kBodyAll, false>(r, j, mci0, mci1);
+      }
+      o.x = maybe_commit<GATED>(mci0, r.c[j].x, GATED ? r.f[j].x : 0);
+      o.y = maybe_commit<GATED>(mci1, r.c[j].y, GATED ? r.f[j].y : 0);
+    }
     even[j] = __ballot(o.x != r.c[j].x);
     odd[j] = __ballot(o.y != r.c[j].y);
     n_changed += __popcll(even[j]) + __popcll(odd[j]);
diff --git a/raftsql_amd/csrc/raftq_step_kernels.hpp b/raftsql_amd/csrc/raftq_step_kernels.hpp
--- a/raftsql_amd/csrc/raftq_step_kernels.hpp
+++ b/raftsql_amd/csrc/raftq_step_kernels.hpp
@@ -236,7 +236,10 @@
     a.rec[g] = r;
     if (committed != committed0) a.committed[g] = committed;
     if (role != role0) a.role[g] = role;
-    if (first_idx != first_idx0) a.first_idx[g] = first_idx;
+    if (first_idx != first_idx0) {
+      a.first_idx[g] = first_idx;
+      if (a.self_max != nullptr && a.self_max[2] != 0u) a.self_max[2] = 0u;
+    }
 #pragma unroll
     for (int p = 0; p < kMaxPeers; ++p)
       if ((mt_dirty >> p) & 1u) a.match[(uint64_t)p * a.ld + g] = mt[p];
diff --git a/raftsql_amd/engine.py b/raftsql_amd/engine.py
--- a/raftsql_amd/engine.py
+++ b/raftsql_amd/engine.py
@@ -374,6 +374,11 @@
         self._chk(self._lib.raftq_narrow_rebuild(self._h))
         return self.narrow()
 
+    def gate_narrow(self) -> bool:
+        v = C.c_int32(0)
+        self._chk(self._lib.raftq_gate_narrow(self._h, C.byref(v)))
+        return bool(v.value)
+
     def read_votes(self) -> np.ndarray:
         out = np.empty((self.n_peers, self.n_groups), dtype=np.uint8)
         self._chk(self._lib.raftq_read_votes(self._h, _ptr(out)))
```

Measured after the change: 129.3 billion (median of 2 runs). About the same (-0.3%).
